# binli123/dsmil-wsi

Measured on NVIDIA H100. Metric: patches/sec DSMIL fwd at N=10k D=512, higher is better.
Workload: dtype f32

## Files before the change

dsmil_wsi_b200/csrc/abi.cu:

```cuda
#include <atomic>
#include <cstdarg>
#include <cstdio>
#include <cstring>
#include <cstdlib>
#include <vector>
#include <algorithm>
#include <climits>

#include "common.cuh"
#include "gemm_generic.cuh"
#include "fwd_kernels.cuh"
#include "bwd_kernels.cuh"
#include "bwd_bags.cuh"
#include "fwd_sm90.cuh"
#include "fwd_batched.cuh"
#include "bag_plan.cuh"
#include "embed_kernels.cuh"
#include "jpeg_kernels.cuh"

namespace dsmil {

static thread_local char g_err[512] = "";
__device__ unsigned long long scratch_keys[kMaxC];
static std::atomic<uint64_t> g_launches{0};

void set_error(const char* fmt, ...) {
  va_list ap;
  va_start(ap, fmt);
  vsnprintf(g_err, sizeof(g_err), fmt, ap);
  va_end(ap);
}
int cuda_fail(cudaError_t e, const char* what) {
  set_error("CUDA error %d (%s) at %s", static_cast<int>(e), cudaGetErrorString(e), what);
  return DSMIL_ERR_CUDA;
}
void count_launch(int n) { g_launches.fetch_add(static_cast<uint64_t>(n), std::memory_order_relaxed); }

__global__ void __launch_bounds__(256)
k_gather_rows(const float* __restrict__ X, int D, const long long* __restrict__ idx, long long M,
              float* __restrict__ out) {
  const int lane = threadIdx.x & 31;
  const long long stride = static_cast<long long>(gridDim.x) * 8;
  const bool vec = (D % 4 == 0) && ((reinterpret_cast<uintptr_t>(X) & 15) == 0) && ((reinterpret_cast<uintptr_t>(out) & 15) == 0);
  for (long long m = static_cast<long long>(blockIdx.x) * 8 + (threadIdx.x >> 5); m < M; m += stride) {
    const float* src = X + idx[m] * D;
    float* dst = out + m * D;
    if (vec) {
      for (int j = lane; j < (D >> 2); j += 32)
        reinterpret_cast<float4*>(dst)[j] = __ldg(reinterpret_cast<const float4*>(src) + j);
    } else {
      for (int j = lane; j < D; j += 32) dst[j] = __ldg(src + j);
    }
  }
}



__global__ void __launch_bounds__(256)
k_u8hwc_to_f32chw(const uint8_t* __restrict__ in, long long B, int H, int W, int Cc, float* __restrict__ out) {
  const long long plane = static_cast<long long>(H) * W;
  const long long total = B * plane;
  const long long stride = static_cast<long long>(gridDim.x) * blockDim.x;
  for (long long i = static_cast<long long>(blockIdx.x) * blockDim.x + threadIdx.x; i < total; i += stride) {
    const long long b = i / plane, px = i % plane;
    const uint8_t* src = in + i * Cc;
    float* dst = out + b * Cc * plane + px;
    for (int c = 0; c < Cc; ++c) dst[c * plane] = __fdiv_rn(static_cast<float>(src[c]), 255.f);
  }
}

bool g_prof_on = false;
struct ProfRec { int tag; cudaEvent_t a, b; };
static std::vector<ProfRec> g_prof;
static std::vector<ProfRec> g_prof_pool;
static int g_prof_open[PROF_NTAGS];
void prof_begin_impl(int tag, cudaStream_t st) {
  if (g_prof.size() >= 16384) { g_prof_open[tag] = -1; return; }
  ProfRec r;
  if (!g_prof_pool.empty()) { r = g_prof_pool.back(); g_prof_pool.pop_back(); }
  else { if (cudaEventCreate(&r.a) != cudaSuccess || cudaEventCreate(&r.b) != cudaSuccess) { g_prof_open[tag] = -1; return; } }
  r.tag = tag;
  cudaEventRecord(r.a, st);
  g_prof_open[tag] = static_cast<int>(g_prof.size());
  g_prof.push_back(r);
}
void prof_end_impl(int tag, cudaStream_t st) {
  const int i = g_prof_open[tag];
  if (i >= 0 && i < static_cast<int>(g_prof.size())) cudaEventRecord(g_prof[i].b, st);
}

static int check_params(const dsmil_params_t* p, bool need_scores = false) {
  DSMIL_REQUIRE(p != nullptr, "params is NULL");
  DSMIL_REQUIRE(!need_scores || (p->Wi && p->bi), "NULL instance-classifier weights");
  DSMIL_REQUIRE(p->D >= 1 && p->D <= DSMIL_MAX_D, "feature size D=%d outside [1,%d]", p->D, DSMIL_MAX_D);
  DSMIL_REQUIRE(p->C >= 1 && p->C <= DSMIL_MAX_C, "output classes C=%d outside [1,%d]", p->C, DSMIL_MAX_C);
  DSMIL_REQUIRE(p->W1 && p->b1 && p->Wf && p->bf, "NULL weight pointer");
  DSMIL_REQUIRE(!p->nonlinear || (p->W2 && p->b2), "nonlinear q needs W2/b2");
  DSMIL_REQUIRE(!p->passing_v || (p->Wv && p->bv), "passing_v needs Wv/bv");
  return 0;
}

static int check_workspace(size_t need, bool ok, const void* ws, size_t cap) {
  if (ws && ok) return 0;
  set_error("workspace too small: need %zu bytes, got %zu", need, cap);
  return DSMIL_ERR_WORKSPACE;
}

static int check_bags(const float* const* Xs, const int64_t* Ns, int nb, int64_t* total, bool* aligned) {
  *total = 0;
  *aligned = true;
  for (int b = 0; b < nb; ++b) {
    DSMIL_REQUIRE(Ns[b] >= 0 && Ns[b] < 0xffffffffll, "bag %d: N=%lld out of range", b, (long long)Ns[b]);
    if (Ns[b] == 0) {
      set_error("bag %d: empty bag (N == 0): the reference raises IndexError at dsmil.py:53", b);
      return DSMIL_ERR_EMPTY;
    }
    if (!Xs) {
      *total += Ns[b];
      continue;
    }
    DSMIL_REQUIRE(Xs[b], "bag %d: NULL features", b);
    *aligned = *aligned && (reinterpret_cast<uintptr_t>(Xs[b]) & 15) == 0;
    *total += Ns[b];
  }
  return 0;
}

static inline int attend_ctas(int64_t N) {
  const int64_t tiles = (N + kAttendRows - 1) / kAttendRows;
  return static_cast<int>(tiles < kSplits ? (tiles < 1 ? 1 : tiles) : kSplits);
}

static int num_sms() {
  static int cached[64] = {0};
  int dev = 0;
  if (cudaGetDevice(&dev) != cudaSuccess || dev < 0 || dev >= 64) return kSms;
  if (!cached[dev]) {
    int n = 0;
    if (cudaDeviceGetAttribute(&n, cudaDevAttrMultiProcessorCount, dev) != cudaSuccess || n <= 0) n = kSms;
    cached[dev] = n;
  }
  return cached[dev];
}

struct Phase1Ws {
  sm90::BagDev* table;
  unsigned long long* keys;
  unsigned int* counters;
  uint8_t* wimg;
};
static void carve_phase1(Carver& c, const dsmil_params_t* p, int nb, Phase1Ws& w) {
  w.table = c.take<sm90::BagDev>(nb);
  w.keys = c.take<unsigned long long>(static_cast<size_t>(nb) * (kMaxC + 1));
  w.counters = reinterpret_cast<unsigned int*>(w.keys ? w.keys + static_cast<size_t>(nb) * kMaxC : nullptr);
  w.wimg = nullptr;
  if (sm90::qmlp_supported(p)) {
    const uintptr_t img = reinterpret_cast<uintptr_t>(c.take<uint8_t>(sm90::wimg_bytes(p->D) + 1024));
    w.wimg = reinterpret_cast<uint8_t*>((img + 1023) & ~uintptr_t(1023));
  }
}

static int build_table(const float* const* Xs, const int64_t* Ns, int nb, std::vector<sm90::BagDev>& tbl, int* tiles,
                       int* recs) {
  long long row = 0;
  int tile = 0, rec = 0;
  tbl.resize(nb);
  for (int b = 0; b < nb; ++b) {
    DSMIL_REQUIRE(Ns[b] >= 1 && Ns[b] < 0xffffffffll && Xs[b], "bag %d: empty or NULL", b);
    DSMIL_REQUIRE((reinterpret_cast<uintptr_t>(Xs[b]) & 15) == 0, "bag %d: features must be 16-byte aligned", b);
    tbl[b] = bag_entry(Xs[b], Ns[b], row, tile, rec);
  }
  *tiles = tile;
  *recs = rec;
  return 0;
}

static int bags_phase1_impl(const dsmil_params_t* p, const Phase1Ws& w, const float* const* Xs, const int64_t* Ns,
                            int nb, const float* classes_in, float* classes, float* Q, float* H1, bool q_blocked,
                            bool upload, int* tiles, int* recs, cudaStream_t st) {
  std::vector<sm90::BagDev> tbl;
  int rc;
  if ((rc = build_table(Xs, Ns, nb, tbl, tiles, recs))) return rc;
  if (upload)
    DSMIL_CUDA_OK(cudaMemcpyAsync(w.table, tbl.data(), sizeof(sm90::BagDev) * nb, cudaMemcpyHostToDevice, st));
  DSMIL_CUDA_OK(cudaMemsetAsync(w.keys, 0, sizeof(unsigned long long) * (kMaxC + 1) * nb, st));
  if (upload && (rc = sm90::launch_prep_wimg(p, w.wimg, st))) return rc;
  if (classes_in) {
    const int grid = static_cast<int>(std::min<int64_t>(ceil_div(Ns[0], 256), kSplits));
    k_argmax<<<grid, 256, 0, st>>>(classes_in, Ns[0], p->C, w.keys);
    DSMIL_LAUNCH_OK("k_argmax");
  }
  return sm90::launch_qmlp(p, w.table, nb, *tiles, classes_in ? nullptr : classes, w.keys, Q, H1, w.wimg, num_sms(),
                           st, q_blocked);
}

struct FwdWs : Phase1Ws {
  float *Q, *H1, *V, *cand, *qmax, *recs, *rec;
  int64_t* crit;
  size_t bytes;
};
static FwdWs carve_fwd(const dsmil_params_t* p, int64_t N, void* ws, size_t cap, bool* ok) {
  Carver c(ws, cap);
  FwdWs w;
  const int64_t n = N > 0 ? N : 1;
  carve_phase1(c, p, 1, w);
  w.Q = c.take<float>(n * kQ);
  w.H1 = p->nonlinear ? c.take<float>(n * kQ) : nullptr;
  w.V = p->passing_v ? c.take<float>(n * p->D) : nullptr;
  w.cand = c.take<float>(cand_floats(p->C));
  w.qmax = c.take<float>(static_cast<size_t>(p->C) * kQ);
  w.crit = c.take<int64_t>(kMaxC);
  w.recs = c.take<float>(static_cast<size_t>(attend_ctas(N)) * rec_floats(p->C, p->D));
  w.rec = c.take<float>(rec_floats(p->C, p->D));
  w.bytes = c.off;
  *ok = c.ok();
  return w;
}


static int launch_scores(const dsmil_params_t* p, const float* X, int64_t N, float* classes,
                         unsigned long long* keys, cudaStream_t st) {
  const int C = p->C, D = p->D;
  const size_t smem = sizeof(float) * C * D;
  const bool vec = (D % 4 == 0) && ((reinterpret_cast<uintptr_t>(X) & 15) == 0);
  const int mode = !vec ? 0 : (D % 64 == 0 ? 2 : 1);
  const int grid = static_cast<int>(std::min<int64_t>(ceil_div(N, mode == 2 ? 64 : 8), kSms * 8));
  prof_begin(PROF_SCORES, st);
  if (mode == 2) {
    if (smem > 48 * 1024) DSMIL_CUDA_OK(cudaFuncSetAttribute(k_scores<2>, cudaFuncAttributeMaxDynamicSharedMemorySize, (int)smem));
    k_scores<2><<<grid, 256, smem, st>>>(X, N, D, p->Wi, p->bi, C, classes, keys);
  } else if (mode == 1) {
    if (smem > 48 * 1024) DSMIL_CUDA_OK(cudaFuncSetAttribute(k_scores<1>, cudaFuncAttributeMaxDynamicSharedMemorySize, (int)smem));
    k_scores<1><<<grid, 256, smem, st>>>(X, N, D, p->Wi, p->bi, C, classes, keys);
  } else {
    if (smem > 48 * 1024) DSMIL_CUDA_OK(cudaFuncSetAttribute(k_scores<0>, cudaFuncAttributeMaxDynamicSharedMemorySize, (int)smem));
    k_scores<0><<<grid, 256, smem, st>>>(X, N, D, p->Wi, p->bi, C, classes, keys);
  }
  prof_end(PROF_SCORES, st);
  DSMIL_LAUNCH_OK("k_scores");
  return 0;
}

static bool stream_is_capturing(cudaStream_t st) {
  cudaStreamCaptureStatus cs = cudaStreamCaptureStatusNone;
  return cudaStreamIsCapturing(st, &cs) == cudaSuccess && cs != cudaStreamCaptureStatusNone;
}

static bool phase1_on_qmlp(const dsmil_params_t* p, const uint8_t* wimg, const float* X) {
  return sm90::qmlp_supported(p) && wimg && (reinterpret_cast<uintptr_t>(X) & 15) == 0;
}

static int phase1_impl(const dsmil_params_t* p, const float* X, const float* xv, const float* classes_in,
                       int64_t N, int64_t row_offset, float* classes, float* Q, float* H1, float* V,
                       float* cand, const Phase1Ws& w, cudaStream_t st) {
  const int C = p->C, D = p->D;
  int rc;
  if (N > 0 && classes_in && classes && classes != classes_in)
    DSMIL_CUDA_OK(cudaMemcpyAsync(classes, classes_in, sizeof(float) * N * C, cudaMemcpyDeviceToDevice, st));
  if (N > 0 && phase1_on_qmlp(p, w.wimg, X)) {
    int tiles, recs;
    if ((rc = bags_phase1_impl(p, w, &X, &N, 1, classes_in, classes, Q, H1, false, true, &tiles, &recs, st))) return rc;
  } else {
    DSMIL_CUDA_OK(cudaMemsetAsync(w.keys, 0, sizeof(unsigned long long) * kMaxC, st));
    if (N > 0) {
      if (classes_in) {
        const int grid = static_cast<int>(std::min<int64_t>(ceil_div(N, 256), kSplits));
        k_argmax<<<grid, 256, 0, st>>>(classes_in, N, C, w.keys);
        DSMIL_LAUNCH_OK("k_argmax");
      } else if ((rc = launch_scores(p, X, N, classes, w.keys, st))) {
        return rc;
      }
      prof_begin(PROF_QMLP, st);
      if (p->nonlinear) {
        if ((rc = launch_linear<ACT_RELU, false>(X, N, D, p->W1, p->b1, kQ, H1, nullptr, 0, st))) return rc;
        if ((rc = launch_linear<ACT_TANH, false>(H1, N, kQ, p->W2, p->b2, kQ, Q, nullptr, 0, st))) return rc;
      } else {
        if ((rc = launch_linear<ACT_NONE, false>(X, N, D, p->W1, p->b1, kQ, Q, nullptr, 0, st))) return rc;
      }
      prof_end(PROF_QMLP, st);
    }
  }
  if (N > 0 && p->passing_v &&
      (rc = launch_linear<ACT_RELU, false>(xv ? xv : X, N, D, p->Wv, p->bv, D, V, nullptr, 0, st)))
    return rc;
  const float* cls = classes_in ? classes_in : classes;
  k_gather_cand<<<C, kQ, 0, st>>>(w.keys, cls, Q, N, C, row_offset, cand);
  DSMIL_LAUNCH_OK("k_gather_cand");
  return 0;
}

__global__ void k_empty_rec(float* rec, int C, int Dv) {
  const size_t n = rec_floats(C, Dv);
  for (size_t i = blockIdx.x * blockDim.x + threadIdx.x; i < n; i += static_cast<size_t>(gridDim.x) * blockDim.x)
    rec[i] = (i < static_cast<size_t>(C)) ? -INFINITY : 0.f;
}

template <int CT>
static int launch_attend_j(int J, int grid, cudaStream_t st, const float* V, int Dv, const float* Q, int64_t N,
                           const float* qmax, int C, float* A, float* recs) {
  switch (J) {
    case 1: k_attend<CT, 1><<<grid, 256, 0, st>>>(V, Dv, Q, N, qmax, C, A, recs); break;
    case 2: k_attend<CT, 2><<<grid, 256, 0, st>>>(V, Dv, Q, N, qmax, C, A, recs); break;
    case 4: k_attend<CT, 4><<<grid, 256, 0, st>>>(V, Dv, Q, N, qmax, C, A, recs); break;
    case 8: k_attend<CT, 8><<<grid, 256, 0, st>>>(V, Dv, Q, N, qmax, C, A, recs); break;
    default: k_attend<CT, 16><<<grid, 256, 0, st>>>(V, Dv, Q, N, qmax, C, A, recs); break;
  }
  DSMIL_LAUNCH_OK("k_attend");
  return 0;
}

static int phase2_impl(const dsmil_params_t* p, const float* V, const float* Q, int64_t N, const float* qmax,
                       float* A, float* rec, float* recs, cudaStream_t st) {
  const int C = p->C, Dv = p->D;
  if (N <= 0) {
    k_empty_rec<<<4, 256, 0, st>>>(rec, C, Dv);
    DSMIL_LAUNCH_OK("k_empty_rec");
    return 0;
  }
  const int grid = attend_ctas(N);
  int j = ceil_div(Dv, 256), J = 1;
  while (J < j) J <<= 1;
  int rc;
  prof_begin(PROF_ATTEND, st);
  if (C == 1) rc = launch_attend_j<1>(J, grid, st, V, Dv, Q, N, qmax, C, A, recs);
  else if (C == 2) rc = launch_attend_j<2>(J, grid, st, V, Dv, Q, N, qmax, C, A, recs);
  else if (C <= 4) rc = launch_attend_j<4>(J, grid, st, V, Dv, Q, N, qmax, C, A, recs);
  else rc = launch_attend_j<8>(J, grid, st, V, Dv, Q, N, qmax, C, A, recs);
  prof_end(PROF_ATTEND, st);
  if (rc) return rc;
  dim3 g2(C, ceil_div(Dv, 256));
  k_combine_rec<<<g2, 256, 0, st>>>(recs, grid, C, Dv, rec);
  DSMIL_LAUNCH_OK("k_combine_rec");
  return 0;
}

static int phase3_impl(const dsmil_params_t* p, int64_t N, const float* rec, float* A, float* B, float* pred,
                       cudaStream_t st) {
  const int grid = static_cast<int>(std::min<int64_t>(std::max<int64_t>(ceil_div(N * p->C, 256), 1), kSplits));
  prof_begin(PROF_FINAL, st);
  k_finalize<<<grid, 256, 0, st>>>(rec, N, p->C, p->D, p->Wf, p->bf, A, B, pred);
  prof_end(PROF_FINAL, st);
  DSMIL_LAUNCH_OK("k_finalize");
  return 0;
}

static int forward_bags_impl(const dsmil_params_t* p, const float* const* Xs, const int64_t* Ns, int nb,
                             const float* classes_in, float* classes, float* pred, float* A, float* B,
                             int64_t* crit, float* save_Q, float* save_H1, void* ws, size_t ws_bytes,
                             cudaStream_t st);

static int forward_impl(const dsmil_params_t* p, const float* X, const float* xv, const float* classes_in,
                        int64_t N, float* classes, float* pred, float* A, float* B, int64_t* crit_idx,
                        float* save_Q, float* save_H1, float* save_V, void* ws, size_t ws_bytes, cudaStream_t st) {
  int rc = check_params(p, classes_in == nullptr);
  if (rc) return rc;
  DSMIL_REQUIRE(N >= 0 && N < 0xffffffffll, "N=%lld out of range", (long long)N);
  if (N == 0) {
    set_error("empty bag (N == 0): the reference raises IndexError at dsmil.py:53");
    return DSMIL_ERR_EMPTY;
  }
  DSMIL_REQUIRE(X && pred && A && B && (classes || classes_in), "NULL tensor pointer");
  if (sm90::batched_supported(p) && (reinterpret_cast<uintptr_t>(X) & 15) == 0)
    return forward_bags_impl(p, &X, &N, 1, classes_in, classes, pred, A, B, crit_idx, save_Q, save_H1, ws, ws_bytes, st);
  bool ok;
  FwdWs w = carve_fwd(p, N, ws, ws_bytes, &ok);
  if ((rc = check_workspace(w.bytes, ok, ws, ws_bytes))) return rc;
  float* Q = save_Q ? save_Q : w.Q;
  float* H1 = p->nonlinear ? (save_H1 ? save_H1 : w.H1) : nullptr;
  float* V = p->passing_v ? (save_V ? save_V : w.V) : nullptr;
  if ((rc = phase1_impl(p, X, xv, classes_in, N, 0, classes, Q, H1, V, w.cand, w, st))) return rc;
  int64_t* crit = crit_idx ? crit_idx : w.crit;
  k_merge_cand<<<p->C, kQ, 0, st>>>(w.cand, 1, 1, p->C, w.qmax, crit);
  DSMIL_LAUNCH_OK("k_merge_cand");
  const float* Vv = p->passing_v ? V : X;
  if ((rc = phase2_impl(p, Vv, Q, N, w.qmax, A, w.rec, w.recs, st))) return rc;
  return phase3_impl(p, N, w.rec, A, B, pred, st);
}


struct BagsWs : Phase1Ws {
  float* Q;
  float* recs;
  float* pred_part;
  long long* row_offsets;
  float* qmax;
  size_t bytes;
};
static BagsWs carve_bags(const dsmil_params_t* p, const int64_t* Ns, int nb, bool need_Q, bool sharded, void* ws,
                         size_t cap, bool* ok) {
  Carver c(ws, cap);
  BagsWs w;
  int64_t tiles = 0, nrec = 0;
  for (int b = 0; b < nb; ++b) {
    tiles += tiles_for_bag(Ns[b]);
    nrec += recs_for_bag(Ns[b]);
  }
  carve_phase1(c, p, nb, w);
  w.pred_part = c.take<float>(static_cast<size_t>(nb) * sm90::kFinSlices * kMaxC);
  w.Q = need_Q ? c.take<float>(static_cast<size_t>(tiles) * sm90::kTileM * kQ) : nullptr;
  w.recs = c.take<float>(static_cast<size_t>(nrec) * rec_floats(p->C, p->D));
  w.row_offsets = sharded ? c.take<long long>(nb) : nullptr;
  w.qmax = sharded ? c.take<float>(static_cast<size_t>(nb) * p->C * kQ) : nullptr;
  w.bytes = c.off;
  *ok = c.ok();
  return w;
}

static int bags_attend_finalize(const dsmil_params_t* p, const BagsWs& w, int nb, const float* Q, bool q_blocked,
                                float* pred, float* A, float* B, int64_t* crit, int recs, const int* recs_dev,
                                cudaStream_t st) {
  const int C = p->C, D = p->D;
  int rc;
  sm90::AttendArgs aa{w.table, nb, D, C, Q, q_blocked, w.keys, A, w.recs, nullptr, recs_dev};
  if ((rc = sm90::launch_attend_b(aa, recs, st))) return rc;
  sm90::FinalizeArgs fa{w.table, D, C, w.recs, w.keys, p->Wf, p->bf, A, B, pred, reinterpret_cast<long long*>(crit),
                         w.pred_part, w.counters, nullptr, 0, 0};
  return sm90::launch_finalize_b(fa, nb, st);
}

static int forward_bags_impl(const dsmil_params_t* p, const float* const* Xs, const int64_t* Ns, int nb,
                             const float* classes_in, float* classes, float* pred, float* A, float* B,
                             int64_t* crit, float* save_Q, float* save_H1, void* ws, size_t ws_bytes,
                             cudaStream_t st) {
  bool ok;
  BagsWs w = carve_bags(p, Ns, nb, save_Q == nullptr, false, ws, ws_bytes, &ok);
  int rc = check_workspace(w.bytes, ok, ws, ws_bytes);
  if (rc) return rc;
  float* Q = save_Q ? save_Q : w.Q;
  const bool q_blocked = save_Q == nullptr;
  int tiles, recs;
  if ((rc = bags_phase1_impl(p, w, Xs, Ns, nb, classes_in, classes, Q, save_H1, q_blocked, true, &tiles, &recs, st)))
    return rc;
  return bags_attend_finalize(p, w, nb, Q, q_blocked, pred, A, B, crit, recs, nullptr, st);
}

}

using namespace dsmil;

extern "C" {

int dsmil_abi_version(void) { return DSMIL_ABI_VERSION; }
const char* dsmil_last_error(void) { return g_err; }
uint64_t dsmil_launch_count(void) { return g_launches.load(std::memory_order_relaxed); }
int dsmil_forward_path(const dsmil_params_t* p, int64_t N) {
  (void)N;
  return (p && p->C >= 1 && p->C <= DSMIL_MAX_C && p->D >= 1 && p->D <= DSMIL_MAX_D && sm90::qmlp_supported(p)) ? 2 : 1;
}


int dsmil_gather_rows(const float* X, int64_t N, int32_t D, const int64_t* idx, int64_t M, float* out, void* stream) {
  DSMIL_REQUIRE(N >= 0 && M >= 0 && D >= 1 && (M == 0 || (X && idx && out)), "bad arguments");
  if (M == 0) return 0;
  const int grid = static_cast<int>(std::min<int64_t>((M + 7) / 8, kSms * 8));
  k_gather_rows<<<grid, 256, 0, static_cast<cudaStream_t>(stream)>>>(X, D, reinterpret_cast<const long long*>(idx), M, out);
  DSMIL_LAUNCH_OK("k_gather_rows");
  return 0;
}

int dsmil_patches_u8_to_f32(const uint8_t* in, int64_t B, int32_t H, int32_t W, int32_t Cc, float* out, void* stream) {
  DSMIL_REQUIRE(B >= 0 && H >= 1 && W >= 1 && Cc >= 1 && Cc <= 4 && (B == 0 || (in && out)), "bad arguments");
  if (B == 0) return 0;
  const long long total = static_cast<long long>(B) * H * W;
  const int grid = static_cast<int>(std::min<long long>((total + 255) / 256, kSms * 16));
  k_u8hwc_to_f32chw<<<grid, 256, 0, static_cast<cudaStream_t>(stream)>>>(in, B, H, W, Cc, out);
  DSMIL_LAUNCH_OK("k_u8hwc_to_f32chw");
  return 0;
}

int dsmil_instnorm_act(const float* x, const float* residual, float* y, int64_t planes, int32_t HW, float eps,
                       int32_t relu, void* stream) {
  DSMIL_REQUIRE(planes >= 0 && HW >= 1 && HW <= kInPlaneMax && eps >= 0.f && (planes == 0 || (x && y)),
                "bad arguments (HW must be in [1, %d])", kInPlaneMax);
  DSMIL_REQUIRE(planes < (1ll << 31), "too many planes");
  if (planes == 0) return 0;
  return launch_instnorm(x, residual, y, planes, HW, eps, relu, static_cast<cudaStream_t>(stream));
}

int dsmil_instnorm_act_nhwc(const float* x, const float* residual, float* y, int64_t N, int32_t HW, int32_t C, float eps,
                            int32_t relu, void* stream) {
  DSMIL_REQUIRE(N >= 0 && HW >= 1 && C >= 32 && C % 32 == 0 && eps >= 0.f && (N == 0 || (x && y)),
                "bad arguments (C must be a multiple of 32)");
  DSMIL_REQUIRE(N * (C / 32) < (1ll << 31), "too many (sample, channel group) slabs");
  if (N == 0) return 0;
  return launch_instnorm_nhwc(x, residual, y, N, HW, C, eps, relu, static_cast<cudaStream_t>(stream));
}

static JpegBatch carve_jpeg(void* ws, size_t cap, int n, int H, int W, int64_t blob_bytes, size_t* need) {
  Carver cv(ws, cap);
  JpegBatch a{};
  a.n = n; a.H = H; a.W = W;
  a.plane_elems = jpeg_plane_elems(H, W);
  a.unstuffed = cv.take<uint8_t>(static_cast<size_t>(blob_bytes) + 64);
  a.coef = cv.take<int16_t>(static_cast<size_t>(3) * a.plane_elems * n);
  a.planes = cv.take<uint8_t>(static_cast<size_t>(3) * a.plane_elems * n);
  *need = cv.off;
  return a;
}

int32_t dsmil_jpeg_header_bytes_dev(void) { return static_cast<int32_t>(sizeof(dsmil_jpeg_header)); }

int64_t dsmil_jpeg_workspace_bytes(int32_t n, int32_t H, int32_t W, int64_t blob_bytes) {
  if (n < 0 || H < 1 || W < 1 || H > 65535 || W > 65535 || blob_bytes < 0) return -1;
  size_t need = 0;
  carve_jpeg(nullptr, 0, n, H, W, blob_bytes, &need);
  return static_cast<int64_t>(need);
}

int dsmil_jpeg_decode_batch(const uint8_t* blob, int64_t blob_bytes, const void* headers, int32_t n, int32_t H, int32_t W,
                            uint8_t* out_u8, float* out_f32, int32_t f32_channels_last, int32_t* status, void* workspace,
                            int64_t workspace_bytes, void* stream) {
  DSMIL_REQUIRE(n >= 0 && H >= 1 && W >= 1 && H <= 65535 && W <= 65535 && blob_bytes >= 0 &&
                (f32_channels_last == 0 || f32_channels_last == 1), "bad arguments");
  if (n == 0) return 0;
  DSMIL_REQUIRE(blob && headers && status && workspace && (out_u8 || out_f32), "null pointer");
  DSMIL_REQUIRE((reinterpret_cast<uintptr_t>(headers) & 15) == 0 && (reinterpret_cast<uintptr_t>(workspace) & 255) == 0 &&
                (out_f32 == nullptr || (reinterpret_cast<uintptr_t>(out_f32) & 15) == 0) &&
                (out_u8 == nullptr || (reinterpret_cast<uintptr_t>(out_u8) & 3) == 0),
                "headers must be 16-byte, workspace 256-byte, out_f32 16-byte, out_u8 4-byte aligned");
  size_t need = 0;
  JpegBatch a = carve_jpeg(workspace, static_cast<size_t>(workspace_bytes), n, H, W, blob_bytes, &need);
  const int rc = check_workspace(need, static_cast<int64_t>(need) <= workspace_bytes, workspace,
                                 static_cast<size_t>(std::max<int64_t>(workspace_bytes, 0)));
  if (rc) return rc;
  a.blob = blob;
  a.hdr = static_cast<const dsmil_jpeg_header*>(headers);
  a.out_u8 = out_u8;
  a.out_f32 = out_f32;
  a.f32_hwc = f32_channels_last;
  a.status = status;
  return launch_jpeg_decode(a, static_cast<cudaStream_t>(stream));
}

int dsmil_profile_enable(int on) {
  g_prof_on = on != 0;
  return 0;
}
int dsmil_profile_read(double* ms_per_tag, uint64_t* launches_per_tag) {
  DSMIL_REQUIRE(ms_per_tag && launches_per_tag, "NULL output");
  for (int t = 0; t < PROF_NTAGS; ++t) { ms_per_tag[t] = 0.0; launches_per_tag[t] = 0; }
  for (auto& r : g_prof) {
    float ms = 0.f;
    if (cudaEventSynchronize(r.b) == cudaSuccess && cudaEventElapsedTime(&ms, r.a, r.b) == cudaSuccess) {
      ms_per_tag[r.tag] += ms;
      launches_per_tag[r.tag] += 1;
    }
    g_prof_pool.push_back(r);
  }
  g_prof.clear();
  cudaGetLastError();
  return 0;
}

size_t dsmil_cand_floats(int32_t C) { return cand_floats(C); }
size_t dsmil_rec_floats(int32_t C, int32_t Dv) { return rec_floats(C, Dv); }

size_t dsmil_forward_workspace_bytes(const dsmil_params_t* p, int64_t N) {
  if (!p || p->C < 1 || p->C > DSMIL_MAX_C || p->D < 1 || p->D > DSMIL_MAX_D || N < 0) return 0;
  bool ok;
  size_t a = carve_fwd(p, N, nullptr, 0, &ok).bytes;
  if (sm90::batched_supported(p) && N > 0) a = std::max(a, carve_bags(p, &N, 1, true, false, nullptr, 0, &ok).bytes);
  return a;
}

size_t dsmil_forward_bags_workspace_bytes(const dsmil_params_t* p, const int64_t* Ns, int32_t nb) {
  if (!p || !Ns || nb < 1 || p->C < 1 || p->C > DSMIL_MAX_C || p->D < 1 || p->D > DSMIL_MAX_D) return 0;
  bool ok;
  int64_t mx = 0;
  for (int b = 0; b < nb; ++b) mx = std::max<int64_t>(mx, Ns[b]);
  size_t bytes = carve_fwd(p, mx, nullptr, 0, &ok).bytes;
  if (sm90::batched_supported(p)) bytes = std::max(bytes, carve_bags(p, Ns, nb, true, false, nullptr, 0, &ok).bytes);
  return bytes;
}

int dsmil_forward_bags(const dsmil_params_t* p, const float* const* Xs, const int64_t* Ns, int32_t nb,
                       float* classes, float* pred, float* A, float* B, int64_t* crit_idx, void* workspace,
                       size_t workspace_bytes, void* stream) {
  int rc = check_params(p, true);
  if (rc) return rc;
  DSMIL_REQUIRE(Xs && Ns && nb >= 1 && classes && pred && A && B, "NULL pointer or nb < 1");
  cudaStream_t st = static_cast<cudaStream_t>(stream);
  int64_t total;
  bool aligned;
  if ((rc = check_bags(Xs, Ns, nb, &total, &aligned))) return rc;
  const size_t need = dsmil_forward_bags_workspace_bytes(p, Ns, nb);
  if ((rc = check_workspace(need, workspace_bytes >= need, workspace, workspace ? workspace_bytes : 0))) return rc;
  if (sm90::batched_supported(p) && aligned)
    return forward_bags_impl(p, Xs, Ns, nb, nullptr, classes, pred, A, B, crit_idx, nullptr, nullptr, workspace,
                             workspace_bytes, st);
  int64_t row = 0;
  for (int b = 0; b < nb; ++b) {
    rc = forward_impl(p, Xs[b], nullptr, nullptr, Ns[b], classes + row * p->C, pred + static_cast<size_t>(b) * p->C,
                      A + row * p->C, B + static_cast<size_t>(b) * p->C * p->D,
                      crit_idx ? crit_idx + static_cast<size_t>(b) * p->C : nullptr, nullptr, nullptr, nullptr,
                      workspace, workspace_bytes, st);
    if (rc) return rc;
    row += Ns[b];
  }
  return 0;
}
size_t dsmil_shard_workspace_bytes(const dsmil_params_t* p, int64_t N_local) {
  return dsmil_forward_workspace_bytes(p, N_local);
}

int dsmil_forward(const dsmil_params_t* p, const float* X, const float* x_for_v, int64_t N, float* classes,
                  float* pred, float* A, float* B, int64_t* crit_idx, float* save_Q, float* save_H1,
                  float* save_V, void* workspace, size_t workspace_bytes, void* stream) {
  DSMIL_REQUIRE(classes != nullptr, "classes is NULL");
  return forward_impl(p, X, x_for_v, nullptr, N, classes, pred, A, B, crit_idx, save_Q, save_H1, save_V,
                      workspace, workspace_bytes, static_cast<cudaStream_t>(stream));
}

int dsmil_bag_forward(const dsmil_params_t* p, const float* X, const float* x_for_v, const float* classes_in,
                      int64_t N, float* pred, float* A, float* B, int64_t* crit_idx, float* save_Q,
                      float* save_H1, float* save_V, void* workspace, size_t workspace_bytes, void* stream) {
  DSMIL_REQUIRE(classes_in != nullptr, "classes_in is NULL");
  return forward_impl(p, X, x_for_v, classes_in, N, nullptr, pred, A, B, crit_idx, save_Q, save_H1, save_V,
                      workspace, workspace_bytes, static_cast<cudaStream_t>(stream));
}

int dsmil_instance_scores(const dsmil_params_t* p, const float* X, int64_t N, float* classes, void* stream) {
  DSMIL_REQUIRE(p && p->Wi && p->bi && p->C >= 1 && p->C <= DSMIL_MAX_C && p->D >= 1 && p->D <= DSMIL_MAX_D,
                "bad params");
  DSMIL_REQUIRE(N >= 0 && (N == 0 || (X && classes)), "NULL tensor pointer");
  if (N == 0) return 0;
  unsigned long long* keys;
  DSMIL_CUDA_OK(cudaGetSymbolAddress(reinterpret_cast<void**>(&keys), scratch_keys));
  return launch_scores(p, X, N, classes, keys, static_cast<cudaStream_t>(stream));
}

int dsmil_shard_phase1(const dsmil_params_t* p, const float* X, const float* x_for_v, const float* classes_in,
                       int64_t N_local, int64_t row_offset, float* classes, float* Q, float* H1, float* V,
                       float* cand_rec, void* workspace, size_t workspace_bytes, void* stream) {
  int rc = check_params(p, classes_in == nullptr);
  if (rc) return rc;
  DSMIL_REQUIRE(N_local >= 0 && N_local < 0xffffffffll, "N_local out of range");
  DSMIL_REQUIRE(cand_rec && (N_local == 0 || (X && Q && (classes || classes_in))), "NULL tensor pointer");
  DSMIL_REQUIRE(N_local == 0 || !p->passing_v || V, "passing_v needs a V buffer");
  bool ok;
  FwdWs w = carve_fwd(p, N_local, workspace, workspace_bytes, &ok);
  if ((rc = check_workspace(w.bytes, ok, workspace, workspace_bytes))) return rc;
  float* h1 = p->nonlinear ? (H1 ? H1 : (phase1_on_qmlp(p, w.wimg, X) ? nullptr : w.H1)) : nullptr;
  return phase1_impl(p, X, x_for_v, classes_in, N_local, row_offset, classes, Q, h1, V, cand_rec, w,
                     static_cast<cudaStream_t>(stream));
}

int dsmil_shard_merge_candidates(int32_t C, const float* cand_recs, int32_t G, float* q_max, int64_t* crit_idx,
                                 void* stream) {
  DSMIL_REQUIRE(C >= 1 && C <= DSMIL_MAX_C && G >= 1 && cand_recs && q_max && crit_idx, "bad arguments");
  k_merge_cand<<<C, kQ, 0, static_cast<cudaStream_t>(stream)>>>(cand_recs, G, 1, C, q_max, crit_idx);
  DSMIL_LAUNCH_OK("k_merge_cand");
  return 0;
}

int dsmil_shard_phase2(const dsmil_params_t* p, const float* Xv, const float* Q, int64_t N_local,
                       const float* q_max, float* A_logits, float* rec, void* workspace, size_t workspace_bytes,
                       void* stream) {
  int rc = check_params(p);
  if (rc) return rc;
  DSMIL_REQUIRE(rec && q_max && (N_local == 0 || (Xv && Q && A_logits)), "NULL tensor pointer");
  bool ok;
  FwdWs w = carve_fwd(p, N_local, workspace, workspace_bytes, &ok);
  if ((rc = check_workspace(w.bytes, ok, workspace, workspace_bytes))) return rc;
  return phase2_impl(p, Xv, Q, N_local, q_max, A_logits, rec, w.recs, static_cast<cudaStream_t>(stream));
}

int dsmil_shard_merge_partials(int32_t C, int32_t Dv, const float* recs, int32_t G, float* rec_out, void* stream) {
  DSMIL_REQUIRE(C >= 1 && C <= DSMIL_MAX_C && Dv >= 1 && G >= 1 && G <= kMaxRecs && recs && rec_out, "bad arguments");
  dim3 g2(C, ceil_div(Dv, 256));
  k_combine_rec<<<g2, 256, 0, static_cast<cudaStream_t>(stream)>>>(recs, G, C, Dv, rec_out);
  DSMIL_LAUNCH_OK("k_combine_rec");
  return 0;
}

int dsmil_shard_phase3(const dsmil_params_t* p, int64_t N_local, const float* rec_global, float* A, float* B,
                       float* pred, void* stream) {
  int rc = check_params(p);
  if (rc) return rc;
  DSMIL_REQUIRE(rec_global && B && pred && (N_local == 0 || A), "NULL tensor pointer");
  return phase3_impl(p, N_local, rec_global, A, B, pred, static_cast<cudaStream_t>(stream));
}

struct BwdWs {
  float *dB, *dA, *tpart, *dqm, *dz2, *dz1, *tnpart, *cspart, *dzv, *tmp;
  size_t bytes;
};
static BwdWs carve_bwd(const dsmil_params_t* p, int64_t N, int need_gX, void* ws, size_t cap, bool* ok) {
  Carver c(ws, cap);
  BwdWs w;
  const int C = p->C, D = p->D;
  const int64_t n = N > 0 ? N : 1;
  w.dB = c.take<float>(static_cast<size_t>(C) * D);
  w.dA = c.take<float>(n * C);
  w.tpart = c.take<float>(kSplits * kMaxC);
  w.dqm = c.take<float>(static_cast<size_t>(C) * kQ);
  w.dz2 = c.take<float>(n * kQ);
  w.dz1 = p->nonlinear ? c.take<float>(n * kQ) : nullptr;
  size_t tn = tn_partial_floats(kQ, D, N);
  tn = std::max(tn, tn_partial_floats(kQ, kQ, N));
  tn = std::max(tn, tn_partial_floats(C, kQ, N));
  tn = std::max(tn, tn_partial_floats(C, D, N));
  if (p->passing_v) tn = std::max(tn, tn_partial_floats(D, D, N));
  w.tnpart = c.take<float>(tn);
  w.cspart = c.take<float>(static_cast<size_t>(kSplits) * std::max(D, kQ));
  w.dzv = p->passing_v ? c.take<float>(n * D) : nullptr;
  w.tmp = (p->passing_v && need_gX) ? c.take<float>(n * D) : nullptr;
  w.bytes = c.off;
  *ok = c.ok();
  return w;
}

size_t dsmil_backward_workspace_bytes(const dsmil_params_t* p, int64_t N, int need_gX) {
  if (!p || p->C < 1 || p->C > DSMIL_MAX_C || p->D < 1 || p->D > DSMIL_MAX_D || N < 0) return 0;
  bool ok;
  return carve_bwd(p, N, need_gX, nullptr, 0, &ok).bytes;
}


static int bwd_phase1_impl(const dsmil_params_t* p, const float* X, const float* Vv, int64_t N, const float* A,
                           const float* B, const float* d_classes, const float* d_pred, const float* d_A,
                           const float* d_B, const dsmil_grads_t* g, float* dA, const BwdWs& w, int* gs,
                           cudaStream_t st) {
  const int C = p->C, D = p->D;
  int rc;
  k_bwd_bag<<<ceil_div(static_cast<int64_t>(C) * D, 256), 256, 0, st>>>(p->Wf, B, d_pred, d_B, C, D, w.dB, g->gWf,
                                                                        g->gbf);
  DSMIL_LAUNCH_OK("k_bwd_bag");
  if (g->gWi) {
    if (d_classes && N > 0) { if ((rc = launch_gemm_tn(d_classes, C, X, D, N, w.tnpart, g->gWi, st))) return rc; }
    else DSMIL_CUDA_OK(cudaMemsetAsync(g->gWi, 0, sizeof(float) * C * D, st));
  }
  if (g->gbi) {
    if (d_classes && N > 0) { if ((rc = launch_colsum(d_classes, C, N, w.cspart, g->gbi, st))) return rc; }
    else DSMIL_CUDA_OK(cudaMemsetAsync(g->gbi, 0, sizeof(float) * C, st));
  }
  *gs = static_cast<int>(std::min<int64_t>(ceil_div(N, 256), kSplits));
  if (N == 0) return 0;
  const size_t smem = sizeof(float) * C * D;
  if (smem > 48 * 1024)
    DSMIL_CUDA_OK(cudaFuncSetAttribute(k_rowdot, cudaFuncAttributeMaxDynamicSharedMemorySize, (int)smem));
  const int grid = static_cast<int>(std::min<int64_t>(ceil_div(N, 8), kSms * 8));
  k_rowdot<<<grid, 256, smem, st>>>(Vv, N, D, w.dB, C, d_A, dA);
  DSMIL_LAUNCH_OK("k_rowdot");
  k_bwd_t_partial<<<*gs, 256, 0, st>>>(A, dA, N, C, w.tpart);
  DSMIL_LAUNCH_OK("k_bwd_t_partial");
  return 0;
}

static int bwd_phase2_impl(const dsmil_params_t* p, int64_t N, const float* A, float* dA, const float* part, int P,
                           const float* Q, float* dqm, const BwdWs& w, cudaStream_t st) {
  if (N > 0) {
    const int gs = static_cast<int>(std::min<int64_t>(ceil_div(N, 256), kSplits));
    k_bwd_dL<<<gs, 256, 0, st>>>(A, dA, N, p->C, part, P);
    DSMIL_LAUNCH_OK("k_bwd_dL");
  }
  return launch_gemm_tn(dA, p->C, Q, kQ, N, w.tnpart, dqm, st);
}

static int bwd_phase3_impl(const dsmil_params_t* p, const float* X, int64_t N, int64_t row_offset, const float* Q,
                           const float* H1, const float* dL, const float* dqm, const float* qmax, const int64_t* crit,
                           const dsmil_grads_t* g, const BwdWs& w, const float** dz1, cudaStream_t st) {
  int rc;
  if (N > 0) {
    const int grid = static_cast<int>(std::min<int64_t>(ceil_div(N * kQ, 256), kSms * 8));
    k_bwd_dq<<<grid, 256, 0, st>>>(dL, Q, qmax, dqm, crit, N, row_offset, p->C, p->nonlinear, w.dz2);
    DSMIL_LAUNCH_OK("k_bwd_dq");
  }
  *dz1 = w.dz2;
  if (p->nonlinear) {
    if (g->gW2 && (rc = launch_gemm_tn(w.dz2, kQ, H1, kQ, N, w.tnpart, g->gW2, st))) return rc;
    if (g->gb2 && (rc = launch_colsum(w.dz2, kQ, N, w.cspart, g->gb2, st))) return rc;
    if (N > 0 && (rc = launch_linear<ACT_MASK_POS, true>(w.dz2, N, kQ, p->W2, nullptr, kQ, w.dz1, H1, 0, st))) return rc;
    *dz1 = w.dz1;
  }
  if (g->gW1 && (rc = launch_gemm_tn(*dz1, kQ, X, p->D, N, w.tnpart, g->gW1, st))) return rc;
  if (g->gb1 && (rc = launch_colsum(*dz1, kQ, N, w.cspart, g->gb1, st))) return rc;
  return 0;
}

int dsmil_backward(const dsmil_params_t* p, const float* X, const float* x_for_v, int64_t N, const float* Q,
                   const float* H1, const float* V, const float* A, const float* B, const int64_t* crit_idx,
                   const float* d_classes, const float* d_pred, const float* d_A, const float* d_B,
                   const dsmil_grads_t* g, const float* v_mask, void* workspace, size_t workspace_bytes,
                   void* stream) {
  int rc = check_params(p);
  if (rc) return rc;
  DSMIL_REQUIRE(N >= 1 && X && Q && A && B && crit_idx && g, "NULL tensor pointer or N < 1");
  DSMIL_REQUIRE(!p->nonlinear || H1, "nonlinear q backward needs saved H1");
  DSMIL_REQUIRE(!p->passing_v || V, "passing_v backward needs saved V");
  cudaStream_t st = static_cast<cudaStream_t>(stream);
  const int C = p->C, D = p->D;
  bool ok;
  BwdWs w = carve_bwd(p, N, g->gX != nullptr, workspace, workspace_bytes, &ok);
  if ((rc = check_workspace(w.bytes, ok, workspace, workspace_bytes))) return rc;
  const float* Xv = x_for_v ? x_for_v : X;
  int gs;
  const float* dz1;
  if ((rc = bwd_phase1_impl(p, X, p->passing_v ? V : X, N, A, B, d_classes, d_pred, d_A, d_B, g, w.dA, w, &gs, st)) ||
      (rc = bwd_phase2_impl(p, N, A, w.dA, w.tpart, gs, Q, w.dqm, w, st)) ||
      (rc = bwd_phase3_impl(p, X, N, 0, Q, H1, w.dA, w.dqm, nullptr, crit_idx, g, w, &dz1, st)))
    return rc;

  const int ge = static_cast<int>(std::min<int64_t>(ceil_div(N * D, 256), kSms * 8));
  if (p->passing_v) {
    k_bwd_dzv<<<ge, 256, 0, st>>>(A, w.dB, V, N, C, D, w.dzv);
    DSMIL_LAUNCH_OK("k_bwd_dzv");
    if (g->gWv && (rc = launch_gemm_tn(w.dzv, D, Xv, D, N, w.tnpart, g->gWv, st))) return rc;
    if (g->gbv && (rc = launch_colsum(w.dzv, D, N, w.cspart, g->gbv, st))) return rc;
  }
  if (g->gX) {
    if ((rc = launch_linear<ACT_NONE, true>(dz1, N, kQ, p->W1, nullptr, D, g->gX, nullptr, 0, st))) return rc;
    k_bwd_dx_extra<<<ge, 256, 0, st>>>(d_classes, p->Wi, p->passing_v ? nullptr : A, w.dB, N, C, D, 1, g->gX);
    DSMIL_LAUNCH_OK("k_bwd_dx_extra");
    if (p->passing_v) {
      if ((rc = launch_linear<ACT_NONE, true>(w.dzv, N, D, p->Wv, nullptr, D, w.tmp, nullptr, 0, st))) return rc;
      k_axpy_mask<<<ge, 256, 0, st>>>(w.tmp, v_mask, N * D, g->gX);
      DSMIL_LAUNCH_OK("k_axpy_mask");
    }
  }
  return 0;
}

int dsmil_shard_backward_phase1(const dsmil_params_t* p, const float* X, int64_t N, const float* A, const float* B,
                                const float* d_classes, const float* d_pred, float* dA, float* t_local, float* gWi,
                                float* gbi, float* gWf, float* gbf, void* workspace, size_t workspace_bytes,
                                void* stream) {
  int rc = check_params(p);
  if (rc) return rc;
  DSMIL_REQUIRE(!p->passing_v, "sharded backward supports the identity v only");
  DSMIL_REQUIRE(N >= 0 && B && t_local && (N == 0 || (X && A && dA)), "NULL tensor pointer or N < 0");
  cudaStream_t st = static_cast<cudaStream_t>(stream);
  bool ok;
  BwdWs w = carve_bwd(p, N, 0, workspace, workspace_bytes, &ok);
  if ((rc = check_workspace(w.bytes, ok, workspace, workspace_bytes))) return rc;
  dsmil_grads_t g{};
  g.gWi = gWi; g.gbi = gbi; g.gWf = gWf; g.gbf = gbf;
  int gs;
  if ((rc = bwd_phase1_impl(p, X, X, N, A, B, d_classes, d_pred, nullptr, nullptr, &g, dA, w, &gs, st))) return rc;
  if (N == 0) {
    DSMIL_CUDA_OK(cudaMemsetAsync(t_local, 0, sizeof(float) * p->C, st));
    return 0;
  }
  return launch_sum_partials(w.tpart, gs, p->C, t_local, st);
}

int dsmil_shard_backward_phase2(const dsmil_params_t* p, int64_t N, const float* A, float* dA, const float* t_global,
                                const float* Q, float* dqm_local, void* workspace, size_t workspace_bytes,
                                void* stream) {
  int rc = check_params(p);
  if (rc) return rc;
  DSMIL_REQUIRE(N >= 0 && t_global && dqm_local && (N == 0 || (A && dA && Q)), "NULL tensor pointer or N < 0");
  bool ok;
  BwdWs w = carve_bwd(p, N, 0, workspace, workspace_bytes, &ok);
  if ((rc = check_workspace(w.bytes, ok, workspace, workspace_bytes))) return rc;
  return bwd_phase2_impl(p, N, A, dA, t_global, 1, Q, dqm_local, w, static_cast<cudaStream_t>(stream));
}

int dsmil_shard_backward_phase3(const dsmil_params_t* p, const float* X, int64_t N, int64_t row_offset, const float* Q,
                                const float* H1, const float* dL, const float* dqm_global, const float* q_max,
                                const int64_t* crit_idx, float* gW1, float* gb1, float* gW2, float* gb2,
                                void* workspace, size_t workspace_bytes, void* stream) {
  int rc = check_params(p);
  if (rc) return rc;
  DSMIL_REQUIRE(N >= 0 && dqm_global && q_max && crit_idx && (N == 0 || (X && Q && dL)), "NULL tensor pointer or N < 0");
  DSMIL_REQUIRE(!p->nonlinear || N == 0 || H1, "nonlinear q backward needs saved H1");
  bool ok;
  BwdWs w = carve_bwd(p, N, 0, workspace, workspace_bytes, &ok);
  if ((rc = check_workspace(w.bytes, ok, workspace, workspace_bytes))) return rc;
  dsmil_grads_t g{};
  g.gW1 = gW1; g.gb1 = gb1; g.gW2 = gW2; g.gb2 = gb2;
  const float* dz1;
  return bwd_phase3_impl(p, X, N, row_offset, Q, H1, dL, dqm_global, q_max, crit_idx, &g, w, &dz1,
                         static_cast<cudaStream_t>(stream));
}

int dsmil_instance_scores_backward(const dsmil_params_t* p, const float* X, int64_t N, const float* d_classes,
                                   float* gWi, float* gbi, float* gX, void* workspace, size_t workspace_bytes,
                                   void* stream) {
  DSMIL_REQUIRE(p && p->Wi && p->C >= 1 && p->C <= DSMIL_MAX_C && p->D >= 1 && p->D <= DSMIL_MAX_D, "bad params");
  DSMIL_REQUIRE(N >= 1 && X && d_classes, "NULL tensor pointer or N < 1");
  cudaStream_t st = static_cast<cudaStream_t>(stream);
  const int C = p->C, D = p->D;
  Carver c(workspace, workspace_bytes);
  float* tnpart = c.take<float>(tn_partial_floats(C, D, N));
  float* cspart = c.take<float>(static_cast<size_t>(kSplits) * kMaxC);
  int rc = check_workspace(c.off, c.ok(), workspace, workspace_bytes);
  if (rc) return rc;
  if (gWi && (rc = launch_gemm_tn(d_classes, C, X, D, N, tnpart, gWi, st))) return rc;
  if (gbi && (rc = launch_colsum(d_classes, C, N, cspart, gbi, st))) return rc;
  if (gX) {
    const int ge = static_cast<int>(std::min<int64_t>(ceil_div(N * D, 256), kSms * 8));
    k_bwd_dx_extra<<<ge, 256, 0, st>>>(d_classes, p->Wi, nullptr, nullptr, N, C, D, 0, gX);
    DSMIL_LAUNCH_OK("k_bwd_dx_extra");
  }
  return 0;
}

struct BwdBagsWs {
  BagsPlan* plan;
  float* zero_row;
  sm90::BagDev* table;
  TnChunk *chi, *ch1;
  float *dB, *dA, *dL, *tpart, *dpart, *dqm, *dz2, *dz1, *tnpart, *cspart;
  long long* row_offsets;
  int G;
  bool gemv_i;
  int nci, nc1;
  int64_t rps_i, rps_1;
  size_t bytes;
};
static void layout_bwd_bags(Carver& c, const dsmil_params_t* p, int nb, int64_t n, int nchi, bool sharded,
                            BwdBagsWs& w) {
  const int C = p->C, D = p->D;
  w.table = c.take<sm90::BagDev>(nb);
  w.chi = c.take<TnChunk>(nchi);
  w.ch1 = c.take<TnChunk>(w.nc1);
  w.dB = c.take<float>(static_cast<size_t>(nb) * C * D);
  w.dA = c.take<float>(n * C);
  w.dL = c.take<float>(n * C);
  w.tpart = c.take<float>(static_cast<size_t>(nb) * w.G * C);
  w.dpart = c.take<float>(static_cast<size_t>(nb) * w.G * C * kQ);
  w.dqm = c.take<float>(static_cast<size_t>(nb) * C * kQ);
  w.dz2 = c.take<float>(n * kQ);
  w.dz1 = p->nonlinear ? c.take<float>(n * kQ) : nullptr;
  size_t tn = static_cast<size_t>(nchi) * C * D;
  tn = std::max(tn, static_cast<size_t>(w.nc1) * kQ * D);
  tn = std::max(tn, tn_partial_floats(kQ, kQ, n));
  w.tnpart = c.take<float>(tn);
  w.cspart = c.take<float>(static_cast<size_t>(kSplits) * kQ);
  w.row_offsets = sharded ? c.take<long long>(nb) : nullptr;
}
static BwdBagsWs carve_bwd_bags(const dsmil_params_t* p, const int64_t* Ns, int nb, bool aligned, bool sharded,
                                void* ws, size_t cap, bool* ok) {
  Carver c(ws, cap);
  BwdBagsWs w;
  const int C = p->C, D = p->D;
  int64_t total = 0, mx = 1;
  for (int b = 0; b < nb; ++b) {
    total += Ns[b];
    mx = std::max<int64_t>(mx, Ns[b]);
  }
  w.plan = nullptr;
  w.zero_row = nullptr;
  w.G = bwd_bags_ctas(nb, mx);
  const bool gemv_ok = tn_use_gemv(C, D);
  w.gemv_i = gemv_ok && aligned;
  const int64_t rps_gemv = rag_rows_per_chunk(C, D, total, true), rps_tile = rag_rows_per_chunk(C, D, total, false);
  const int nci_gemv = gemv_ok ? rag_chunks(nullptr, Ns, nb, D, rps_gemv, nullptr) : 0;
  const int nci_tile = rag_chunks(nullptr, Ns, nb, D, rps_tile, nullptr);
  w.rps_i = w.gemv_i ? rps_gemv : rps_tile;
  w.nci = w.gemv_i ? nci_gemv : nci_tile;
  w.rps_1 = rag_rows_per_chunk(kQ, D, total, false);
  w.nc1 = rag_chunks(nullptr, Ns, nb, D, w.rps_1, nullptr);
  layout_bwd_bags(c, p, nb, std::max<int64_t>(total, 1), std::max(nci_gemv, nci_tile), sharded, w);
  w.bytes = c.off;
  *ok = c.ok();
  return w;
}
static BwdBagsWs carve_bwd_bags_dev(const dsmil_params_t* p, int nb, int64_t max_rows, void* ws, size_t cap,
                                    bool* ok) {
  Carver c(ws, cap);
  BwdBagsWs w;
  const int C = p->C, D = p->D;
  w.G = bwd_bags_ctas(nb, max_rows);
  w.gemv_i = tn_use_gemv(C, D);
  w.nci = rag_chunks_cap(C, D, w.gemv_i, nb);
  w.nc1 = rag_chunks_cap(kQ, D, false, nb);
  w.rps_i = w.rps_1 = 0;
  layout_bwd_bags(c, p, nb, static_cast<int64_t>(nb) * max_rows, w.nci, false, w);
  w.plan = c.take<BagsPlan>(1);
  w.zero_row = c.take<float>(D);
  w.bytes = c.off;
  *ok = c.ok();
  return w;
}


static int bwd_bags_phase1_impl(const dsmil_params_t* p, const float* const* Xs, const int64_t* Ns, int nb,
                                int64_t total, const float* A, const float* B, const float* d_classes,
                                const float* d_pred, const float* d_A, const float* d_B, const dsmil_grads_t* g,
                                float* dA, const BwdBagsWs& w, cudaStream_t st) {
  const int C = p->C, D = p->D;
  const BagsPlan* pl = w.plan;
  int rc;
  if (!pl) {
    std::vector<sm90::BagDev> tbl(nb);
    long long row = 0;
    for (int b = 0; b < nb; ++b) {
      tbl[b] = sm90::BagDev{Xs[b], Ns[b], row, 0, 0, 0, 0};
      row += Ns[b];
    }
    std::vector<TnChunk> chi(w.nci), ch1(w.nc1);
    rag_chunks(Xs, Ns, nb, D, w.rps_i, chi.data());
    rag_chunks(Xs, Ns, nb, D, w.rps_1, ch1.data());
    DSMIL_CUDA_OK(cudaMemcpyAsync(w.table, tbl.data(), sizeof(sm90::BagDev) * nb, cudaMemcpyHostToDevice, st));
    DSMIL_CUDA_OK(cudaMemcpyAsync(w.chi, chi.data(), sizeof(TnChunk) * w.nci, cudaMemcpyHostToDevice, st));
    DSMIL_CUDA_OK(cudaMemcpyAsync(w.ch1, ch1.data(), sizeof(TnChunk) * w.nc1, cudaMemcpyHostToDevice, st));
  }

  k_bwd_bag_b<<<ceil_div(static_cast<int64_t>(C) * D, 256), 256, 0, st>>>(p->Wf, B, d_pred, d_B, nb, C, D, w.dB,
                                                                          g->gWf, g->gbf);
  DSMIL_LAUNCH_OK("k_bwd_bag_b");
  if (g->gWi) {
    if (d_classes) {
      if ((rc = launch_gemm_tn_rag(d_classes, C, D, w.chi, w.nci, w.gemv_i, w.tnpart, g->gWi, st, pl ? &pl->nci : nullptr)))
        return rc;
    }
    else DSMIL_CUDA_OK(cudaMemsetAsync(g->gWi, 0, sizeof(float) * C * D, st));
  }
  if (g->gbi) {
    if (d_classes) { if ((rc = launch_colsum(d_classes, C, total, w.cspart, g->gbi, st, pl ? &pl->cs : nullptr))) return rc; }
    else DSMIL_CUDA_OK(cudaMemsetAsync(g->gbi, 0, sizeof(float) * C, st));
  }
  const size_t smem = sizeof(float) * C * D;
  if (smem > 48 * 1024)
    DSMIL_CUDA_OK(cudaFuncSetAttribute(k_bwd_rowdot_b, cudaFuncAttributeMaxDynamicSharedMemorySize, (int)smem));
  k_bwd_rowdot_b<<<dim3(w.G, nb), 256, smem, st>>>(w.table, D, w.dB, C, A, d_A, dA, w.tpart, pl ? &pl->G : nullptr);
  DSMIL_LAUNCH_OK("k_bwd_rowdot_b");
  return 0;
}

static int bwd_bags_phase2_impl(const dsmil_params_t* p, int nb, const float* A, const float* dA, const float* tpart,
                                int P, const float* Q, float* dL, float* dqm, const BwdBagsWs& w, cudaStream_t st) {
  const int C = p->C;
  const int* G_dev = w.plan ? &w.plan->G : nullptr;
  k_bwd_dL_b<<<dim3(w.G, nb), 256, 0, st>>>(w.table, C, A, dA, tpart, P, Q, dL, w.dpart, G_dev);
  DSMIL_LAUNCH_OK("k_bwd_dL_b");
  k_sum_segments<<<dim3(ceil_div(C * kQ, 256), nb), 256, 0, st>>>(w.dpart, w.G, C * kQ, dqm, G_dev);
  DSMIL_LAUNCH_OK("k_sum_segments");
  return 0;
}

static int bwd_bags_phase3_impl(const dsmil_params_t* p, int nb, int64_t total, const float* Q, const float* H1,
                                const float* dL, const float* dqm, const float* qmax, const int64_t* crit,
                                const long long* row_offsets, const dsmil_grads_t* g, const BwdBagsWs& w,
                                const float** dz1, cudaStream_t st) {
  const int D = p->D;
  const BagsPlan* pl = w.plan;
  int rc;
  k_bwd_dq_b<<<dim3(w.G, nb), 256, 0, st>>>(w.table, p->C, dL, Q, qmax, dqm, crit, row_offsets, p->nonlinear, w.dz2);
  DSMIL_LAUNCH_OK("k_bwd_dq_b");
  *dz1 = w.dz2;
  if (p->nonlinear) {
    if (g->gW2 && (rc = launch_gemm_tn(w.dz2, kQ, H1, kQ, total, w.tnpart, g->gW2, st, pl ? &pl->tn2 : nullptr)))
      return rc;
    if (g->gb2 && (rc = launch_colsum(w.dz2, kQ, total, w.cspart, g->gb2, st, pl ? &pl->cs : nullptr))) return rc;
    if ((rc = launch_linear<ACT_MASK_POS, true>(w.dz2, total, kQ, p->W2, nullptr, kQ, w.dz1, H1, 0, st,
                                                pl ? &pl->total : nullptr)))
      return rc;
    *dz1 = w.dz1;
  }
  if (g->gW1 &&
      (rc = launch_gemm_tn_rag(*dz1, kQ, D, w.ch1, w.nc1, false, w.tnpart, g->gW1, st, pl ? &pl->nc1 : nullptr)))
    return rc;
  if (g->gb1 && (rc = launch_colsum(*dz1, kQ, total, w.cspart, g->gb1, st, pl ? &pl->cs : nullptr))) return rc;
  return 0;
}

static int backward_bags_run(const dsmil_params_t* p, const float* const* Xs, const int64_t* Ns, int nb, int64_t total,
                             const float* Q, const float* H1, const float* A, const float* B, const int64_t* crit,
                             const float* d_classes, const float* d_pred, const float* d_A, const float* d_B,
                             const dsmil_grads_t* g, const BwdBagsWs& w, cudaStream_t st) {
  const int C = p->C, D = p->D;
  int rc;
  const float* dz1;
  if ((rc = bwd_bags_phase1_impl(p, Xs, Ns, nb, total, A, B, d_classes, d_pred, d_A, d_B, g, w.dA, w, st)) ||
      (rc = bwd_bags_phase2_impl(p, nb, A, w.dA, w.tpart, w.G, Q, w.dL, w.dqm, w, st)) ||
      (rc = bwd_bags_phase3_impl(p, nb, total, Q, H1, w.dL, w.dqm, nullptr, crit, nullptr, g, w, &dz1, st)))
    return rc;
  if (g->gX) {
    if ((rc = launch_linear<ACT_NONE, true>(dz1, total, kQ, p->W1, nullptr, D, g->gX, nullptr, 0, st))) return rc;
    k_bwd_dx_extra_b<<<dim3(w.G, nb), 256, 0, st>>>(w.table, d_classes, p->Wi, A, w.dB, C, D, g->gX);
    DSMIL_LAUNCH_OK("k_bwd_dx_extra_b");
  }
  return 0;
}

static int backward_bags_impl(const dsmil_params_t* p, const float* const* Xs, const int64_t* Ns, int nb,
                              int64_t total, bool aligned, const float* Q, const float* H1, const float* A,
                              const float* B, const int64_t* crit, const float* d_classes, const float* d_pred,
                              const float* d_A, const float* d_B, const dsmil_grads_t* g, void* ws, size_t ws_bytes,
                              cudaStream_t st) {
  bool ok;
  BwdBagsWs w = carve_bwd_bags(p, Ns, nb, aligned, false, ws, ws_bytes, &ok);
  int rc = check_workspace(w.bytes, ok, ws, ws_bytes);
  if (rc) return rc;
  return backward_bags_run(p, Xs, Ns, nb, total, Q, H1, A, B, crit, d_classes, d_pred, d_A, d_B, g, w, st);
}

int dsmil_shard_bags_supported(const dsmil_params_t* p) {
  return (p && p->C >= 1 && p->C <= DSMIL_MAX_C && p->D >= 1 && p->D <= DSMIL_MAX_D && sm90::batched_supported(p)) ? 1 : 0;
}
size_t dsmil_shard_bags_workspace_bytes(const dsmil_params_t* p, const int64_t* Ns, int32_t nb) {
  if (!dsmil_shard_bags_supported(p) || !Ns || nb < 1) return 0;
  bool ok;
  return carve_bags(p, Ns, nb, true, true, nullptr, 0, &ok).bytes;
}
static int shard_bags_phase1_impl(const dsmil_params_t* p, const float* const* Xs, const int64_t* Ns, int nb,
                                  const int64_t* row_offsets, float* classes, float* Q, float* H1, bool q_blocked,
                                  float* cand_recs, const BagsWs& w, cudaStream_t st) {
  const bool upload = !stream_is_capturing(st);
  int tiles, recs, rc;
  if ((rc = bags_phase1_impl(p, w, Xs, Ns, nb, nullptr, classes, Q, H1, q_blocked, upload, &tiles, &recs, st)))
    return rc;
  if (upload)
    DSMIL_CUDA_OK(cudaMemcpyAsync(w.row_offsets, row_offsets, sizeof(long long) * nb, cudaMemcpyHostToDevice, st));
  sm90::k_gather_cand_b<<<dim3(p->C, nb), kQ, 0, st>>>(w.table, w.keys, classes, Q, q_blocked, w.row_offsets, p->C,
                                                        cand_recs);
  DSMIL_LAUNCH_OK("k_gather_cand_b");
  return 0;
}
static int shard_bags_phase2_impl(const dsmil_params_t* p, const float* const* Xs, const int64_t* Ns, int nb,
                                  const float* Q, bool q_blocked, const float* cands_all, int G, float* A,
                                  int64_t* crit_idx, float* qmax, float* recs_out, const BagsWs& w, cudaStream_t st) {
  std::vector<sm90::BagDev> tbl;
  int tiles = 0, recs = 0, rc;
  if ((rc = build_table(Xs, Ns, nb, tbl, &tiles, &recs))) return rc;
  k_merge_cand<<<dim3(p->C, nb), kQ, 0, st>>>(cands_all, G, nb, p->C, qmax, crit_idx);
  DSMIL_LAUNCH_OK("k_merge_cand");
  sm90::AttendArgs aa{w.table, nb, p->D, p->C, Q, q_blocked, w.keys, A, w.recs, qmax, nullptr};
  if ((rc = sm90::launch_attend_b(aa, recs, st))) return rc;
  sm90::FinalizeArgs fa{w.table, p->D, p->C, w.recs, w.keys, p->Wf, p->bf, A, nullptr, nullptr, nullptr,
                         w.pred_part, w.counters, recs_out, 0, 0};
  return sm90::launch_finalize_b(fa, nb, st);
}

int dsmil_shard_bags_phase1(const dsmil_params_t* p, const float* const* Xs, const int64_t* Ns, int32_t nb,
                            const int64_t* row_offsets, float* classes, float* cand_recs, void* workspace,
                            size_t workspace_bytes, void* stream) {
  int rc = check_params(p, true);
  if (rc) return rc;
  DSMIL_REQUIRE(dsmil_shard_bags_supported(p), "shape not supported by the batched tensor-core path");
  DSMIL_REQUIRE(Xs && Ns && nb >= 1 && row_offsets && classes && cand_recs, "NULL pointer or nb < 1");
  bool ok;
  BagsWs w = carve_bags(p, Ns, nb, true, true, workspace, workspace_bytes, &ok);
  if ((rc = check_workspace(w.bytes, ok, workspace, workspace_bytes))) return rc;
  return shard_bags_phase1_impl(p, Xs, Ns, nb, row_offsets, classes, w.Q, nullptr, true, cand_recs, w,
                                static_cast<cudaStream_t>(stream));
}
int dsmil_shard_bags_phase2(const dsmil_params_t* p, const float* const* Xs, const int64_t* Ns, int32_t nb,
                            const float* cands_all, int32_t G, float* A, int64_t* crit_idx, float* recs_out,
                            void* workspace, size_t workspace_bytes, void* stream) {
  int rc = check_params(p, true);
  if (rc) return rc;
  DSMIL_REQUIRE(dsmil_shard_bags_supported(p) && Xs && Ns && nb >= 1 && cands_all && G >= 1 && A && crit_idx && recs_out,
                "bad arguments");
  bool ok;
  BagsWs w = carve_bags(p, Ns, nb, true, true, workspace, workspace_bytes, &ok);
  if ((rc = check_workspace(w.bytes, ok, workspace, workspace_bytes))) return rc;
  return shard_bags_phase2_impl(p, Xs, Ns, nb, w.Q, true, cands_all, G, A, crit_idx, w.qmax, recs_out, w,
                                static_cast<cudaStream_t>(stream));
}
int dsmil_shard_bags_phase3(const dsmil_params_t* p, const float* const* Xs, const int64_t* Ns, int32_t nb,
                            const float* recs_all, int32_t G, float* A, float* B, float* pred, void* workspace,
                            size_t workspace_bytes, void* stream) {
  int rc = check_params(p, true);
  if (rc) return rc;
  DSMIL_REQUIRE(dsmil_shard_bags_supported(p) && Xs && Ns && nb >= 1 && recs_all && G >= 1 && G <= sm90::kMaxRecPerBag && A && B && pred,
                "bad arguments");
  cudaStream_t st = static_cast<cudaStream_t>(stream);
  bool ok;
  BagsWs w = carve_bags(p, Ns, nb, true, true, workspace, workspace_bytes, &ok);
  if ((rc = check_workspace(w.bytes, ok, workspace, workspace_bytes))) return rc;
  sm90::FinalizeArgs fa{w.table, p->D, p->C, recs_all, w.keys, p->Wf, p->bf, A, B, pred, nullptr,
                         w.pred_part, w.counters, nullptr, G, nb};
  return sm90::launch_finalize_b(fa, nb, st);
}


size_t dsmil_forward_bags_train_workspace_bytes(const dsmil_params_t* p, const int64_t* Ns, int32_t nb) {
  if (!p || p->passing_v) return 0;
  return dsmil_forward_bags_workspace_bytes(p, Ns, nb);
}

int dsmil_forward_bags_train(const dsmil_params_t* p, const float* const* Xs, const int64_t* Ns, int32_t nb,
                             float* classes, float* pred, float* A, float* B, int64_t* crit_idx, float* save_Q,
                             float* save_H1, void* workspace, size_t workspace_bytes, void* stream) {
  int rc = check_params(p, true);
  if (rc) return rc;
  DSMIL_REQUIRE(!p->passing_v, "batched training supports the identity v only (passing_v: one bag per call)");
  DSMIL_REQUIRE(Xs && Ns && nb >= 1 && classes && pred && A && B && crit_idx && save_Q && (!p->nonlinear || save_H1),
                "NULL pointer or nb < 1");
  cudaStream_t st = static_cast<cudaStream_t>(stream);
  int64_t total;
  bool aligned;
  if ((rc = check_bags(Xs, Ns, nb, &total, &aligned))) return rc;
  const size_t need = dsmil_forward_bags_train_workspace_bytes(p, Ns, nb);
  if ((rc = check_workspace(need, workspace_bytes >= need, workspace, workspace ? workspace_bytes : 0))) return rc;
  if (sm90::batched_supported(p) && aligned)
    return forward_bags_impl(p, Xs, Ns, nb, nullptr, classes, pred, A, B, crit_idx, save_Q, save_H1, workspace,
                             workspace_bytes, st);
  int64_t row = 0;
  for (int b = 0; b < nb; ++b) {
    rc = forward_impl(p, Xs[b], nullptr, nullptr, Ns[b], classes + row * p->C, pred + static_cast<size_t>(b) * p->C,
                      A + row * p->C, B + static_cast<size_t>(b) * p->C * p->D, crit_idx + static_cast<size_t>(b) * p->C,
                      save_Q + row * kQ, save_H1 ? save_H1 + row * kQ : nullptr, nullptr, workspace, workspace_bytes,
                      st);
    if (rc) return rc;
    row += Ns[b];
  }
  return 0;
}

size_t dsmil_backward_bags_workspace_bytes(const dsmil_params_t* p, const int64_t* Ns, int32_t nb, int need_gX) {
  (void)need_gX;
  if (!p || !Ns || nb < 1 || p->passing_v || p->C < 1 || p->C > DSMIL_MAX_C || p->D < 1 || p->D > DSMIL_MAX_D) return 0;
  for (int b = 0; b < nb; ++b)
    if (Ns[b] < 0) return 0;
  bool ok;
  return carve_bwd_bags(p, Ns, nb, true, false, nullptr, 0, &ok).bytes;
}

int dsmil_backward_bags(const dsmil_params_t* p, const float* const* Xs, const int64_t* Ns, int32_t nb,
                        const float* Q, const float* H1, const float* A, const float* B, const int64_t* crit_idx,
                        const float* d_classes, const float* d_pred, const float* d_A, const float* d_B,
                        const dsmil_grads_t* grads, void* workspace, size_t workspace_bytes, void* stream) {
  int rc = check_params(p);
  if (rc) return rc;
  DSMIL_REQUIRE(!p->passing_v, "batched backward supports the identity v only (passing_v: dsmil_backward per bag)");
  DSMIL_REQUIRE(Xs && Ns && nb >= 1 && nb <= 65535 && Q && A && B && crit_idx && grads,
                "NULL pointer or nb outside [1, 65535]");
  DSMIL_REQUIRE(!p->nonlinear || H1, "nonlinear q backward needs saved H1");
  DSMIL_REQUIRE(!(grads->gX && d_classes) || p->Wi, "gX through d_classes needs Wi");
  int64_t total;
  bool aligned;
  if ((rc = check_bags(Xs, Ns, nb, &total, &aligned))) return rc;
  const size_t need = dsmil_backward_bags_workspace_bytes(p, Ns, nb, grads->gX != nullptr);
  if ((rc = check_workspace(need, workspace_bytes >= need, workspace, workspace ? workspace_bytes : 0))) return rc;
  return backward_bags_impl(p, Xs, Ns, nb, total, aligned, Q, H1, A, B, crit_idx, d_classes, d_pred, d_A, d_B, grads,
                            workspace, workspace_bytes, static_cast<cudaStream_t>(stream));
}


static int check_shard_bags_train(const dsmil_params_t* p, bool need_scores, const float* const* Xs, bool need_X,
                                  const int64_t* Ns, int nb, int64_t* total, bool* aligned) {
  int rc = check_params(p, need_scores);
  if (rc) return rc;
  DSMIL_REQUIRE(!p->passing_v, "row-sharded batched training supports the identity v only");
  DSMIL_REQUIRE(dsmil_shard_bags_supported(p), "shape not supported by the batched tensor-core path");
  DSMIL_REQUIRE(Ns && (Xs || !need_X) && nb >= 1 && nb <= 65535, "NULL pointer or nb outside [1, 65535]");
  return check_bags(need_X ? Xs : nullptr, Ns, nb, total, aligned);
}

int dsmil_shard_bags_phase1_train(const dsmil_params_t* p, const float* const* Xs, const int64_t* Ns, int32_t nb,
                                  const int64_t* row_offsets, float* classes, float* save_Q, float* save_H1,
                                  float* cand_recs, void* workspace, size_t workspace_bytes, void* stream) {
  int64_t total;
  bool aligned;
  int rc = check_shard_bags_train(p, true, Xs, true, Ns, nb, &total, &aligned);
  if (rc) return rc;
  DSMIL_REQUIRE(row_offsets && classes && save_Q && save_H1 && cand_recs, "NULL pointer");
  bool ok;
  BagsWs w = carve_bags(p, Ns, nb, true, true, workspace, workspace_bytes, &ok);
  if ((rc = check_workspace(w.bytes, ok, workspace, workspace_bytes))) return rc;
  return shard_bags_phase1_impl(p, Xs, Ns, nb, row_offsets, classes, save_Q, save_H1, false, cand_recs, w,
                                static_cast<cudaStream_t>(stream));
}

int dsmil_shard_bags_phase2_train(const dsmil_params_t* p, const float* const* Xs, const int64_t* Ns, int32_t nb,
                                  const float* Q, const float* cands_all, int32_t G, float* A, int64_t* crit_idx,
                                  float* q_max, float* recs_out, void* workspace, size_t workspace_bytes,
                                  void* stream) {
  int64_t total;
  bool aligned;
  int rc = check_shard_bags_train(p, true, Xs, true, Ns, nb, &total, &aligned);
  if (rc) return rc;
  DSMIL_REQUIRE(Q && cands_all && G >= 1 && A && crit_idx && q_max && recs_out, "NULL pointer or G < 1");
  bool ok;
  BagsWs w = carve_bags(p, Ns, nb, true, true, workspace, workspace_bytes, &ok);
  if ((rc = check_workspace(w.bytes, ok, workspace, workspace_bytes))) return rc;
  return shard_bags_phase2_impl(p, Xs, Ns, nb, Q, false, cands_all, G, A, crit_idx, q_max, recs_out, w,
                                static_cast<cudaStream_t>(stream));
}

size_t dsmil_shard_backward_bags_workspace_bytes(const dsmil_params_t* p, const int64_t* Ns, int32_t nb) {
  if (!dsmil_shard_bags_supported(p) || !Ns || nb < 1) return 0;
  for (int b = 0; b < nb; ++b)
    if (Ns[b] < 0) return 0;
  bool ok;
  return carve_bwd_bags(p, Ns, nb, true, true, nullptr, 0, &ok).bytes;
}

int dsmil_shard_backward_bags_phase1(const dsmil_params_t* p, const float* const* Xs, const int64_t* Ns, int32_t nb,
                                     const float* A, const float* B, const float* d_classes_local,
                                     const float* d_pred, float* dA_local, float* t_local, float* gWi, float* gbi,
                                     float* gWf, float* gbf, void* workspace, size_t workspace_bytes, void* stream) {
  int64_t total;
  bool aligned;
  int rc = check_shard_bags_train(p, false, Xs, true, Ns, nb, &total, &aligned);
  if (rc) return rc;
  DSMIL_REQUIRE(A && B && dA_local && t_local, "NULL tensor pointer");
  cudaStream_t st = static_cast<cudaStream_t>(stream);
  bool ok;
  BwdBagsWs w = carve_bwd_bags(p, Ns, nb, aligned, true, workspace, workspace_bytes, &ok);
  if ((rc = check_workspace(w.bytes, ok, workspace, workspace_bytes))) return rc;
  dsmil_grads_t g{};
  g.gWi = gWi; g.gbi = gbi; g.gWf = gWf; g.gbf = gbf;
  if ((rc = bwd_bags_phase1_impl(p, Xs, Ns, nb, total, A, B, d_classes_local, d_pred, nullptr, nullptr, &g, dA_local,
                                 w, st)))
    return rc;
  k_sum_segments<<<dim3(ceil_div(p->C, 256), nb), 256, 0, st>>>(w.tpart, w.G, p->C, t_local, nullptr);
  DSMIL_LAUNCH_OK("k_sum_segments");
  return 0;
}

int dsmil_shard_backward_bags_phase2(const dsmil_params_t* p, const int64_t* Ns, int32_t nb, const float* A,
                                     float* dA_to_dL, const float* t_global, const float* Q, float* dqm_local,
                                     void* workspace, size_t workspace_bytes, void* stream) {
  int64_t total;
  bool aligned;
  int rc = check_shard_bags_train(p, false, nullptr, false, Ns, nb, &total, &aligned);
  if (rc) return rc;
  DSMIL_REQUIRE(A && dA_to_dL && t_global && Q && dqm_local, "NULL tensor pointer");
  cudaStream_t st = static_cast<cudaStream_t>(stream);
  bool ok;
  BwdBagsWs w = carve_bwd_bags(p, Ns, nb, true, true, workspace, workspace_bytes, &ok);
  if ((rc = check_workspace(w.bytes, ok, workspace, workspace_bytes))) return rc;
  DSMIL_CUDA_OK(cudaMemcpyAsync(w.dA, dA_to_dL, sizeof(float) * total * p->C, cudaMemcpyDeviceToDevice, st));
  return bwd_bags_phase2_impl(p, nb, A, w.dA, t_global, 1, Q, dA_to_dL, dqm_local, w, st);
}

int dsmil_shard_backward_bags_phase3(const dsmil_params_t* p, const float* const* Xs, const int64_t* Ns, int32_t nb,
                                     const int64_t* row_offsets, const float* Q, const float* H1, const float* dL_local,
                                     const float* dqm_global, const float* q_max, const int64_t* crit_idx,
                                     float* gW1, float* gb1, float* gW2, float* gb2, void* workspace,
                                     size_t workspace_bytes, void* stream) {
  int64_t total;
  bool aligned;
  int rc = check_shard_bags_train(p, false, Xs, true, Ns, nb, &total, &aligned);
  if (rc) return rc;
  DSMIL_REQUIRE(row_offsets && Q && H1 && dL_local && dqm_global && q_max && crit_idx, "NULL tensor pointer");
  cudaStream_t st = static_cast<cudaStream_t>(stream);
  bool ok;
  BwdBagsWs w = carve_bwd_bags(p, Ns, nb, aligned, true, workspace, workspace_bytes, &ok);
  if ((rc = check_workspace(w.bytes, ok, workspace, workspace_bytes))) return rc;
  DSMIL_CUDA_OK(cudaMemcpyAsync(w.row_offsets, row_offsets, sizeof(long long) * nb, cudaMemcpyHostToDevice, st));
  dsmil_grads_t g{};
  g.gW1 = gW1; g.gb1 = gb1; g.gW2 = gW2; g.gb2 = gb2;
  const float* dz1;
  return bwd_bags_phase3_impl(p, nb, total, Q, H1, dL_local, dqm_global, q_max, crit_idx, w.row_offsets, &g, w, &dz1,
                              st);
}


static int check_bags_dev(const dsmil_params_t* p, bool need_scores, const float* const* Xs, const int64_t* Ns, int nb,
                          int64_t max_rows, const int32_t* status) {
  int rc = check_params(p, need_scores);
  if (rc) return rc;
  DSMIL_REQUIRE(dsmil_shard_bags_supported(p),
                "shape not supported by the batched tensor-core path (D=%d, C=%d, nonlinear=%d, passing_v=%d)", p->D,
                p->C, p->nonlinear, p->passing_v);
  DSMIL_REQUIRE(Xs && Ns && status, "NULL bag list or status");
  DSMIL_REQUIRE(nb >= 1 && nb <= 65535, "nb=%d outside [1, 65535]", nb);
  DSMIL_REQUIRE(max_rows >= 1 && max_rows < 0xffffffffll &&
                static_cast<int64_t>(nb) * ((max_rows + sm90::kTileM - 1) / sm90::kTileM) <= INT_MAX,
                "max_rows=%lld out of range for nb=%d", (long long)max_rows, nb);
  return 0;
}

static BagsWs carve_bags_dev(const dsmil_params_t* p, int nb, int64_t max_rows, void* ws, size_t cap, bool* ok,
                             BagsPlan** plan, float** zero_row) {
  const std::vector<int64_t> Ns(nb, max_rows);
  BagsWs w = carve_bags(p, Ns.data(), nb, false, false, ws, cap, ok);
  Carver c(ws, cap);
  c.off = w.bytes;
  *plan = c.take<BagsPlan>(1);
  *zero_row = c.take<float>(p->D);
  w.bytes = c.off;
  *ok = c.ok();
  return w;
}

size_t dsmil_forward_bags_train_dev_workspace_bytes(const dsmil_params_t* p, int32_t nb, int64_t max_rows) {
  if (!dsmil_shard_bags_supported(p) || nb < 1 || nb > 65535 || max_rows < 1 || max_rows >= 0xffffffffll) return 0;
  bool ok;
  BagsPlan* plan;
  float* zero_row;
  const size_t dev = carve_bags_dev(p, nb, max_rows, nullptr, 0, &ok, &plan, &zero_row).bytes;
  const std::vector<int64_t> Ns(nb, max_rows);
  return std::max(dev, dsmil_forward_bags_train_workspace_bytes(p, Ns.data(), nb));
}

int dsmil_forward_bags_train_dev(const dsmil_params_t* p, const float* const* Xs_dev, const int64_t* Ns_dev,
                                 int32_t nb, int64_t max_rows, float* classes, float* pred, float* A, float* B,
                                 int64_t* crit_idx, float* save_Q, float* save_H1, int32_t* status, void* workspace,
                                 size_t workspace_bytes, void* stream) {
  int rc = check_bags_dev(p, true, Xs_dev, Ns_dev, nb, max_rows, status);
  if (rc) return rc;
  DSMIL_REQUIRE(classes && pred && A && B && crit_idx && save_Q && save_H1, "NULL output pointer");
  const size_t need = dsmil_forward_bags_train_dev_workspace_bytes(p, nb, max_rows);
  if ((rc = check_workspace(need, workspace_bytes >= need, workspace, workspace ? workspace_bytes : 0))) return rc;
  cudaStream_t st = static_cast<cudaStream_t>(stream);
  bool ok;
  BagsPlan* plan;
  float* zero_row;
  BagsWs w = carve_bags_dev(p, nb, max_rows, workspace, workspace_bytes, &ok, &plan, &zero_row);
  k_plan_bags<<<1, 32, 0, st>>>(Xs_dev, Ns_dev, nb, max_rows, p->C, p->D, zero_row, w.table, nullptr, nullptr, plan,
                                status);
  DSMIL_LAUNCH_OK("k_plan_bags");
  DSMIL_CUDA_OK(cudaMemsetAsync(w.keys, 0, sizeof(unsigned long long) * (kMaxC + 1) * nb, st));
  if ((rc = sm90::launch_prep_wimg(p, w.wimg, st))) return rc;
  if ((rc = sm90::launch_qmlp(p, w.table, nb, nb * tiles_for_bag(max_rows), classes, w.keys, save_Q, save_H1, w.wimg,
                              num_sms(), st, false, &plan->tiles)))
    return rc;
  return bags_attend_finalize(p, w, nb, save_Q, false, pred, A, B, crit_idx, nb * recs_for_bag(max_rows), &plan->recs,
                              st);
}

size_t dsmil_backward_bags_dev_workspace_bytes(const dsmil_params_t* p, int32_t nb, int64_t max_rows) {
  if (!dsmil_shard_bags_supported(p) || nb < 1 || nb > 65535 || max_rows < 1 || max_rows >= 0xffffffffll) return 0;
  bool ok;
  return carve_bwd_bags_dev(p, nb, max_rows, nullptr, 0, &ok).bytes;
}

int dsmil_backward_bags_dev(const dsmil_params_t* p, const float* const* Xs_dev, const int64_t* Ns_dev, int32_t nb,
                            int64_t max_rows, const float* Q, const float* H1, const float* A, const float* B,
                            const int64_t* crit_idx, const float* d_classes, const float* d_pred, const float* d_A,
                            const float* d_B, const dsmil_grads_t* grads, int32_t* status, void* workspace,
                            size_t workspace_bytes, void* stream) {
  int rc = check_bags_dev(p, false, Xs_dev, Ns_dev, nb, max_rows, status);
  if (rc) return rc;
  DSMIL_REQUIRE(Q && H1 && A && B && crit_idx && grads, "NULL pointer");
  DSMIL_REQUIRE(!d_A && !d_B && !grads->gX,
                "the dev backward takes gradients through classes and pred only (no d_A, d_B or gX)");
  const size_t need = dsmil_backward_bags_dev_workspace_bytes(p, nb, max_rows);
  if ((rc = check_workspace(need, workspace_bytes >= need, workspace, workspace ? workspace_bytes : 0))) return rc;
  cudaStream_t st = static_cast<cudaStream_t>(stream);
  bool ok;
  BwdBagsWs w = carve_bwd_bags_dev(p, nb, max_rows, workspace, workspace_bytes, &ok);
  k_plan_bags<<<1, 32, 0, st>>>(Xs_dev, Ns_dev, nb, max_rows, p->C, p->D, w.zero_row, w.table, w.chi, w.ch1, w.plan,
                                status);
  DSMIL_LAUNCH_OK("k_plan_bags");
  return backward_bags_run(p, nullptr, nullptr, nb, static_cast<int64_t>(nb) * max_rows, Q, H1, A, B, crit_idx,
                           d_classes, d_pred, nullptr, nullptr, grads, w, st);
}

}
```

dsmil_wsi_b200/csrc/fwd_batched.cuh:

```cuda
#pragma once
#include "common.cuh"
#include "fwd_kernels.cuh"
#include "fwd_sm90.cuh"

namespace dsmil {
namespace sm90 {

constexpr int kAttRows = 128;
constexpr int kMaxRecPerBag = 128;

struct AttendArgs {
  const BagDev* bags;
  int nb;
  int D, C;
  const float* Q;
  bool q_blocked;
  const unsigned long long* keys;
  float* A;
  float* recs;
  const float* qmax_ext;
  const int* nrec_dev;
};

template <int CT, int NJ>
__global__ void __launch_bounds__(256, (NJ == 1 && CT <= 2) ? 5 : 0)
k_attend_b(const AttendArgs a) {
  extern __shared__ __align__(16) float s_dyn[];
  __shared__ __align__(16) float sq[CT][kQ];
  __shared__ float sL[kAttRows][CT];
  __shared__ float sE[kAttRows][CT];
  __shared__ float s_red[8][CT];
  const int tid = threadIdx.x, lane = tid & 31, warp = tid >> 5;
  const int C = a.C, D = a.D;
  if (a.nrec_dev != nullptr && static_cast<int>(blockIdx.x) >= *a.nrec_dev) return;
  const int rec = blockIdx.x;
  int bag = 0;
  while (bag < a.nb - 1 && rec >= a.bags[bag + 1].rec_off) ++bag;
  const BagDev bg = a.bags[bag];
  const int cta_in_bag = rec - bg.rec_off;
  const int ntiles = static_cast<int>((bg.N + kAttRows - 1) / kAttRows);

  for (int i = tid; i < CT * kQ; i += 256) {
    const int k = i / kQ, j = i % kQ;
    float v = 0.f;
    if (k < C && a.qmax_ext != nullptr) {
      v = a.qmax_ext[(static_cast<size_t>(bag) * C + k) * kQ + j];
    } else if (k < C) {
      const long long row = key_row(a.keys[static_cast<size_t>(bag) * kMaxC + k]);
      v = a.q_blocked ? tanh_ex2(a.Q[static_cast<size_t>(bg.tile_off + row / kAttRows) * (kAttRows * kQ) + j * kAttRows + (row % kAttRows)])
                      : a.Q[(bg.row_off + row) * kQ + j];
    }
    sq[k][j] = v;
  }
  float run_m[CT], run_s[CT];
#pragma unroll
  for (int k = 0; k < CT; ++k) { run_m[k] = -INFINITY; run_s[k] = 0.f; }
  float acc[CT][NJ][4];
#pragma unroll
  for (int k = 0; k < CT; ++k)
#pragma unroll
    for (int j = 0; j < NJ; ++j)
#pragma unroll
      for (int e = 0; e < 4; ++e) acc[k][j][e] = 0.f;
  __syncthreads();

  const int half = tid >> 7, c4 = tid & 127;
  const int D4 = D >> 2;
  for (int t = cta_in_bag; t < ntiles; t += bg.nrec) {
    const long long r0 = static_cast<long long>(t) * kAttRows;
    const int rows = static_cast<int>((bg.N - r0) < kAttRows ? (bg.N - r0) : kAttRows);
    float Lr[CT];
#pragma unroll
    for (int k = 0; k < CT; ++k) Lr[k] = -INFINITY;
    if (a.q_blocked) {
      const int r = tid & 127, hf = tid >> 7;
      const float* qb = a.Q + static_cast<size_t>(bg.tile_off + t) * (kAttRows * kQ) + static_cast<size_t>(hf * 64) * kAttRows + r;
      float d[CT];
#pragma unroll
      for (int k = 0; k < CT; ++k) d[k] = 0.f;
#pragma unroll 4
      for (int c = 0; c < 64; c += 4) {
        const float* qc = qb + c * kAttRows;
        const f2 ta = fast_tanh2(f2{__ldg(qc), __ldg(qc + kAttRows)});
        const f2 tb = fast_tanh2(f2{__ldg(qc + 2 * kAttRows), __ldg(qc + 3 * kAttRows)});
#pragma unroll
        for (int k = 0; k < CT; ++k) {
          const float4 w = *reinterpret_cast<const float4*>(&sq[k][hf * 64 + c]);
          d[k] = fmaf(ta.x, w.x, d[k]); d[k] = fmaf(ta.y, w.y, d[k]); d[k] = fmaf(tb.x, w.z, d[k]); d[k] = fmaf(tb.y, w.w, d[k]);
        }
      }
      if (hf == 1) {
#pragma unroll
        for (int k = 0; k < CT; ++k) sE[r][k] = d[k];
      }
      __syncthreads();
      if (hf == 0 && r < rows) {
#pragma unroll
        for (int k = 0; k < CT; ++k) {
          Lr[k] = __fdiv_rn(d[k] + sE[r][k], kScale);
          if (k < C) a.A[(bg.row_off + r0 + r) * C + k] = Lr[k];
        }
      }
    } else {
#pragma unroll 4
      for (int rr = 0; rr < 16; ++rr) {
        const int r = warp * 16 + rr;
        if (r < rows) {
          const float4 q = __ldg(reinterpret_cast<const float4*>(a.Q + (bg.row_off + r0 + r) * kQ) + lane);
#pragma unroll
          for (int k = 0; k < CT; ++k) {
            const float4 w = *reinterpret_cast<const float4*>(&sq[k][lane * 4]);
            float d = q.x * w.x;
            d = fmaf(q.y, w.y, d);
            d = fmaf(q.z, w.z, d);
            d = fmaf(q.w, w.w, d);
            d = warp_sum(d);
            if (lane == 0) {
              const float L = __fdiv_rn(d, kScale);
              sL[r][k] = L;
              if (k < C) a.A[(bg.row_off + r0 + r) * C + k] = L;
            }
          }
        }
      }
      __syncthreads();
      if (tid < rows) {
#pragma unroll
        for (int k = 0; k < CT; ++k) Lr[k] = sL[tid][k];
      }
    }
#pragma unroll
    for (int k = 0; k < CT; ++k) {
      const float v = warp_max(Lr[k]);
      if (lane == 0) s_red[warp][k] = v;
    }
    __syncthreads();
    float mnew[CT], scl[CT], ev[CT];
#pragma unroll
    for (int k = 0; k < CT; ++k) {
      float mx = fmaxf(fmaxf(s_red[0][k], s_red[1][k]), fmaxf(s_red[2][k], s_red[3][k]));
      mnew[k] = fmaxf(run_m[k], mx);
      scl[k] = (run_m[k] == -INFINITY) ? 0.f : expf(run_m[k] - mnew[k]);
      ev[k] = (Lr[k] == -INFINITY) ? 0.f : expf(Lr[k] - mnew[k]);
      if (tid < kAttRows) sE[tid][k] = ev[k];
    }
    __syncthreads();
#pragma unroll
    for (int k = 0; k < CT; ++k) {
      const float v = warp_sum(ev[k]);
      if (lane == 0) s_red[warp][k] = v;
    }
    __syncthreads();
#pragma unroll
    for (int k = 0; k < CT; ++k) {
      run_s[k] = run_s[k] * scl[k] + ((s_red[0][k] + s_red[1][k]) + (s_red[2][k] + s_red[3][k]));
      run_m[k] = mnew[k];
    }
#pragma unroll
    for (int k = 0; k < CT; ++k) {
#pragma unroll
      for (int j = 0; j < NJ; ++j)
#pragma unroll
        for (int e = 0; e < 4; ++e) acc[k][j][e] *= scl[k];
    }
    const float* xb = bg.X + r0 * D;
#pragma unroll 8
    for (int r = half; r < rows; r += 2) {
      float4 x[NJ];
#pragma unroll
      for (int j = 0; j < NJ; ++j) {
        const int col = c4 + 128 * j;
        x[j] = col < D4 ? ldg_stream(reinterpret_cast<const float4*>(xb + static_cast<long long>(r) * D) + col)
                        : make_float4(0.f, 0.f, 0.f, 0.f);
      }
#pragma unroll
      for (int k = 0; k < CT; ++k) {
        const float e = sE[r][k];
#pragma unroll
        for (int j = 0; j < NJ; ++j) {
          acc[k][j][0] = fmaf(e, x[j].x, acc[k][j][0]);
          acc[k][j][1] = fmaf(e, x[j].y, acc[k][j][1]);
          acc[k][j][2] = fmaf(e, x[j].z, acc[k][j][2]);
          acc[k][j][3] = fmaf(e, x[j].w, acc[k][j][3]);
        }
      }
    }
    __syncthreads();
  }
  float* recp = a.recs + static_cast<size_t>(rec) * rec_floats(C, D);
  if (half == 1) {
#pragma unroll
    for (int k = 0; k < CT; ++k)
      if (k < C)
#pragma unroll
        for (int j = 0; j < NJ; ++j) {
          const int col = c4 + 128 * j;
          if (col < D4)
            *reinterpret_cast<float4*>(s_dyn + k * D + col * 4) =
                make_float4(acc[k][j][0], acc[k][j][1], acc[k][j][2], acc[k][j][3]);
        }
  }
  __syncthreads();
  if (half == 0) {
#pragma unroll
    for (int k = 0; k < CT; ++k)
      if (k < C)
#pragma unroll
        for (int j = 0; j < NJ; ++j) {
          const int col = c4 + 128 * j;
          if (col < D4) {
            const float4 o = *reinterpret_cast<const float4*>(s_dyn + k * D + col * 4);
            float* dst = recp + 2 * C + static_cast<size_t>(k) * D + col * 4;
            dst[0] = acc[k][j][0] + o.x;
            dst[1] = acc[k][j][1] + o.y;
            dst[2] = acc[k][j][2] + o.z;
            dst[3] = acc[k][j][3] + o.w;
          }
        }
  }
  if (tid == 0) {
#pragma unroll
    for (int k = 0; k < CT; ++k)
      if (k < C) { recp[k] = run_m[k]; recp[C + k] = run_s[k]; }
  }
}

struct FinalizeArgs {
  const BagDev* bags;
  int D, C;
  const float* recs;
  const unsigned long long* keys;
  const float* Wf;
  const float* bf;
  float* A;
  float* B;
  float* pred;
  long long* crit;
  float* pred_part;
  unsigned int* counters;
  float* emit;
  int ext_P, ext_nb;
};

constexpr int kFinSlices = 32;

__global__ void __launch_bounds__(256, 4)
k_finalize_b(const FinalizeArgs a) {
  __shared__ float sw[kMaxRecPerBag][kMaxC];
  __shared__ float sM[kMaxC], sS[kMaxC];
  __shared__ float s_part[8][32];
  __shared__ float red[kMaxC];
  __shared__ unsigned int s_last;
  const int tid = threadIdx.x, lane = tid & 31, warp = tid >> 5;
  const int C = a.C, D = a.D;
  const int bag = blockIdx.y;
  const BagDev bg = a.bags[bag];
  const size_t rstride = rec_floats(C, D);
  const bool ext = a.ext_P > 0;
  const float* recs = ext ? a.recs + static_cast<size_t>(bag) * rstride : a.recs + static_cast<size_t>(bg.rec_off) * rstride;
  const size_t pstride = ext ? rstride * a.ext_nb : rstride;
  const int P = ext ? a.ext_P : bg.nrec;
  for (int k = warp; k < C; k += 8) {
    float m = -INFINITY;
    for (int p = lane; p < P; p += 32) m = fmaxf(m, recs[p * pstride + k]);
    m = warp_max(m);
    float sacc = 0.f;
    for (int p = lane; p < P; p += 32) {
      const float mp = recs[p * pstride + k];
      const float w = (mp == -INFINITY) ? 0.f : expf(mp - m);
      sw[p][k] = w;
      sacc = fmaf(recs[p * pstride + C + k], w, sacc);
    }
    sacc = warp_sum(sacc);
    if (lane == 0) { sM[k] = m; sS[k] = sacc; }
  }
  __syncthreads();
  if (a.emit == nullptr) {
    const long long total = bg.N * C;
    const long long per = (total + gridDim.x - 1) / gridDim.x;
    const long long lo = per * blockIdx.x, hi = (lo + per) < total ? (lo + per) : total;
    float* Ab = a.A + bg.row_off * C;
    for (long long i = lo + tid; i < hi; i += 256) {
      const int k = static_cast<int>(i % C);
      Ab[i] = __fdiv_rn(expf(Ab[i] - sM[k]), sS[k]);
    }
  }
  const int CD = C * D;
  const int eps = (CD + kFinSlices - 1) / kFinSlices;
  const int e_lo = eps * blockIdx.x, e_hi = (e_lo + eps) < CD ? (e_lo + eps) : CD;
  const int rp = tid >> 5;
  float ppart[kMaxC];
#pragma unroll
  for (int k = 0; k < kMaxC; ++k) ppart[k] = 0.f;
  for (int base = e_lo; base < e_hi; base += 32) {
    const int e = base + lane;
    float acc = 0.f;
    if (e < e_hi) {
      const int k = e / D;
      const float* col = recs + 2 * C + e;
#pragma unroll 1
      for (int p0 = rp; p0 < P; p0 += 64) {
        float v[8];
#pragma unroll
        for (int u = 0; u < 8; ++u) v[u] = (p0 + 8 * u < P) ? col[static_cast<size_t>(p0 + 8 * u) * pstride] : 0.f;
#pragma unroll
        for (int u = 0; u < 8; ++u)
          if (p0 + 8 * u < P) acc = fmaf(v[u], sw[p0 + 8 * u][k], acc);
      }
    }
    s_part[rp][lane] = acc;
    __syncthreads();
    if (rp == 0 && e < e_hi) {
      float tot = s_part[0][lane];
#pragma unroll
      for (int r = 1; r < 8; ++r) tot += s_part[r][lane];
      if (a.emit != nullptr) {
        a.emit[static_cast<size_t>(bag) * rstride + 2 * C + e] = tot;
      } else {
        const int k = e / D;
        const float bval = __fdiv_rn(tot, sS[k]);
        a.B[static_cast<size_t>(bag) * CD + e] = bval;
        for (int kk = 0; kk < C; ++kk) ppart[kk] = fmaf(__ldg(a.Wf + static_cast<size_t>(kk) * CD + e), bval, ppart[kk]);
      }
    }
    __syncthreads();
  }
  if (a.emit != nullptr) {
    if (blockIdx.x == 0 && tid < C) {
      a.emit[static_cast<size_t>(bag) * rstride + tid] = sM[tid];
      a.emit[static_cast<size_t>(bag) * rstride + C + tid] = sS[tid];
    }
    return;
  }
  if (warp == 0) {
    for (int kk = 0; kk < C; ++kk) {
      const float v = warp_sum(ppart[kk]);
      if (lane == 0) red[kk] = v;
    }
  }
  __syncthreads();
  float* part = a.pred_part + (static_cast<size_t>(bag) * kFinSlices + blockIdx.x) * kMaxC;
  if (tid < C) part[tid] = red[tid];
  __threadfence();
  __syncthreads();
  if (tid == 0) s_last = atomicAdd(a.counters + bag, 1u);
  __syncthreads();
  if (s_last != kFinSlices - 1) return;
  __threadfence();
  if (tid < C) {
    const volatile float* pp = a.pred_part + static_cast<size_t>(bag) * kFinSlices * kMaxC;
    float sacc = 0.f;
    for (int sl = 0; sl < kFinSlices; ++sl) sacc += pp[sl * kMaxC + tid];
    a.pred[static_cast<size_t>(bag) * C + tid] = sacc + __ldg(a.bf + tid);
    if (a.crit) a.crit[static_cast<size_t>(bag) * C + tid] = key_row(a.keys[static_cast<size_t>(bag) * kMaxC + tid]);
  }
}

__global__ void __launch_bounds__(128)
k_gather_cand_b(const BagDev* __restrict__ bags, const unsigned long long* __restrict__ keys,
                const float* __restrict__ classes, const float* __restrict__ Q, bool q_blocked,
                const long long* __restrict__ row_offsets, int C, float* __restrict__ cands) {
  const int k = blockIdx.x, bag = blockIdx.y;
  const BagDev bg = bags[bag];
  float* cand = cands + static_cast<size_t>(bag) * cand_floats(C);
  long long* idx = reinterpret_cast<long long*>(cand);
  float* score = cand + 2 * C;
  float* qrow = cand + 3 * C + static_cast<size_t>(k) * kQ;
  const unsigned long long key = keys[static_cast<size_t>(bag) * kMaxC + k];
  if (bg.N <= 0 || key == 0ull) {
    if (threadIdx.x == 0) { idx[k] = INT64_MAX; score[k] = -INFINITY; }
    qrow[threadIdx.x] = 0.f;
    return;
  }
  const long long row = key_row(key);
  if (threadIdx.x == 0) {
    idx[k] = row + row_offsets[bag];
    score[k] = classes[(bg.row_off + row) * C + k];
  }
  qrow[threadIdx.x] = q_blocked
      ? tanh_ex2(Q[static_cast<size_t>(bg.tile_off + row / kAttRows) * (kAttRows * kQ) + threadIdx.x * kAttRows + (row % kAttRows)])
      : Q[(bg.row_off + row) * kQ + threadIdx.x];
}

inline bool batched_supported(const dsmil_params_t* p) {
  return qmlp_supported(p) && !p->passing_v && p->D % 4 == 0 && p->D <= 2048 && p->C <= 4 &&
         ((p->C <= 2) || p->D <= 1024);
}

inline int launch_attend_b(const AttendArgs& a, int nrecs, cudaStream_t st) {
  const int C = a.C, D = a.D;
  const size_t smem = sizeof(float) * C * D;
  const int NJ = D <= 512 ? 1 : (D <= 1024 ? 2 : 4);
  auto go = [&](auto kern) -> int {
    if (smem > 48 * 1024)
      DSMIL_CUDA_OK(cudaFuncSetAttribute(kern, cudaFuncAttributeMaxDynamicSharedMemorySize, static_cast<int>(smem)));
    prof_begin(PROF_ATTEND, st);
    kern<<<nrecs, 256, smem, st>>>(a);
    prof_end(PROF_ATTEND, st);
    DSMIL_LAUNCH_OK("k_attend_b");
    return 0;
  };
  if (C == 1) { if (NJ == 1) return go(k_attend_b<1, 1>); if (NJ == 2) return go(k_attend_b<1, 2>); return go(k_attend_b<1, 4>); }
  if (C == 2) { if (NJ == 1) return go(k_attend_b<2, 1>); if (NJ == 2) return go(k_attend_b<2, 2>); return go(k_attend_b<2, 4>); }
  if (NJ == 1) return go(k_attend_b<4, 1>);
  return go(k_attend_b<4, 2>);
}

inline int launch_finalize_b(const FinalizeArgs& a, int nb, cudaStream_t st) {
  prof_begin(PROF_FINAL, st);
  k_finalize_b<<<dim3(kFinSlices, nb), 256, 0, st>>>(a);
  prof_end(PROF_FINAL, st);
  DSMIL_LAUNCH_OK("k_finalize_b");
  return 0;
}

}
}
```

dsmil_wsi_b200/csrc/fwd_sm90.cuh:

```cuda
#pragma once
#include <cuda_bf16.h>
#include <cstdlib>

#include "common.cuh"

namespace dsmil {
namespace sm90 {

constexpr int kTileM = 128;
constexpr int kChunkK = 64;
constexpr int kTileBytes = kQ * kChunkK * 2;
constexpr int kChunkBytes = 2 * kTileBytes;
constexpr int kWStages = 4;
constexpr int kPrefetchChunks = 2;
constexpr int kConsumerWGs = 2;
constexpr int kWarpProd = 4 * kConsumerWGs;
constexpr int kThreads = 128 * (kConsumerWGs + 1);
constexpr int kRegsConsumer = 232, kRegsProducer = 40;
template <int R> __device__ __forceinline__ void reg_inc() { asm volatile("setmaxnreg.inc.sync.aligned.u32 %0;" ::"n"(R)); }
template <int R> __device__ __forceinline__ void reg_dec() { asm volatile("setmaxnreg.dec.sync.aligned.u32 %0;" ::"n"(R)); }

__device__ __forceinline__ float4 lds128(uint32_t addr) {
  float4 v;
  asm volatile("ld.shared.v4.f32 {%0,%1,%2,%3}, [%4];" : "=f"(v.x), "=f"(v.y), "=f"(v.z), "=f"(v.w) : "r"(addr));
  return v;
}
__device__ __forceinline__ float4 ldg_stream(const float4* p) {
  float4 v;
  asm volatile("ld.global.nc.L1::no_allocate.v4.f32 {%0,%1,%2,%3}, [%4];"
               : "=f"(v.x), "=f"(v.y), "=f"(v.z), "=f"(v.w) : "l"(p));
  return v;
}
__device__ __forceinline__ void prefetch_l2(const void* p) { asm volatile("prefetch.global.L2 [%0];" ::"l"(p)); }

__device__ __forceinline__ uint32_t smem_u32(const void* p) { return static_cast<uint32_t>(__cvta_generic_to_shared(p)); }
__device__ __forceinline__ void mbar_init(uint32_t bar, uint32_t count) {
  asm volatile("mbarrier.init.shared::cta.b64 [%0], %1;" ::"r"(bar), "r"(count));
}
__device__ __forceinline__ void mbar_arrive(uint32_t bar) {
  asm volatile("mbarrier.arrive.shared::cta.b64 _, [%0];" ::"r"(bar) : "memory");
}
__device__ __forceinline__ void mbar_expect_tx(uint32_t bar, uint32_t bytes) {
  asm volatile("mbarrier.arrive.expect_tx.shared::cta.b64 _, [%0], %1;" ::"r"(bar), "r"(bytes) : "memory");
}
__device__ __forceinline__ void mbar_wait(uint32_t bar, uint32_t parity, uint32_t sleep_ns = 0) {
  uint32_t done = 0, spins = 0;
  while (true) {
    asm volatile(
        "{\n\t.reg .pred p;\n\t"
        "mbarrier.try_wait.parity.shared::cta.b64 p, [%1], %2;\n\t"
        "selp.u32 %0, 1, 0, p;\n\t}"
        : "=r"(done) : "r"(bar), "r"(parity) : "memory");
    if (done) break;
    if (sleep_ns) __nanosleep(sleep_ns);
    if (++spins > (1u << 26)) __trap();
  }
}
__device__ __forceinline__ void bulk_g2s(uint32_t dst, const void* src, uint32_t bytes, uint32_t bar) {
  asm volatile("cp.async.bulk.shared::cluster.global.mbarrier::complete_tx::bytes [%0], [%1], %2, [%3];"
               ::"r"(dst), "l"(src), "r"(bytes), "r"(bar) : "memory");
}

__device__ __forceinline__ uint64_t smem_desc(uint32_t saddr) {
  return static_cast<uint64_t>(((saddr & 0x3ffffu) >> 4) | (1u << 16)) |
         (static_cast<uint64_t>((1024u >> 4) | (1u << 30)) << 32);
}
__device__ __forceinline__ void wg_fence() { asm volatile("wgmma.fence.sync.aligned;" ::: "memory"); }
__device__ __forceinline__ void wg_commit() { asm volatile("wgmma.commit_group.sync.aligned;" ::: "memory"); }
__device__ __forceinline__ void wg_wait0() { asm volatile("wgmma.wait_group.sync.aligned 0;" ::: "memory"); }
__device__ __forceinline__ void fence_acc(float (&d)[64]) {
#pragma unroll
  for (int i = 0; i < 64; ++i) asm volatile("" : "+f"(d[i])::"memory");
}
__device__ __forceinline__ void mma_rs(float (&d)[64], uint32_t a0, uint32_t a1, uint32_t a2, uint32_t a3, uint64_t b,
                                       uint32_t acc) {
  asm volatile(
      "{\n\t.reg .pred p;\n\tsetp.ne.b32 p, %68, 0;\n\t"
      "wgmma.mma_async.sync.aligned.m64n128k16.f32.bf16.bf16 "
      "{%0, %1, %2, %3, %4, %5, %6, %7, %8, %9, %10, %11, %12, %13, %14, %15, %16, %17, %18, %19, %20, %21, %22, %23, "
      "%24, %25, %26, %27, %28, %29, %30, %31, %32, %33, %34, %35, %36, %37, %38, %39, %40, %41, %42, %43, %44, %45, "
      "%46, %47, %48, %49, %50, %51, %52, %53, %54, %55, %56, %57, %58, %59, %60, %61, %62, %63}, "
      "{%64, %65, %66, %67}, %69, p, 1, 1, 0;\n\t}"
      : "+f"(d[0]), "+f"(d[1]), "+f"(d[2]), "+f"(d[3]), "+f"(d[4]), "+f"(d[5]), "+f"(d[6]), "+f"(d[7]), "+f"(d[8]),
        "+f"(d[9]), "+f"(d[10]), "+f"(d[11]), "+f"(d[12]), "+f"(d[13]), "+f"(d[14]), "+f"(d[15]), "+f"(d[16]),
        "+f"(d[17]), "+f"(d[18]), "+f"(d[19]), "+f"(d[20]), "+f"(d[21]), "+f"(d[22]), "+f"(d[23]), "+f"(d[24]),
        "+f"(d[25]), "+f"(d[26]), "+f"(d[27]), "+f"(d[28]), "+f"(d[29]), "+f"(d[30]), "+f"(d[31]), "+f"(d[32]),
        "+f"(d[33]), "+f"(d[34]), "+f"(d[35]), "+f"(d[36]), "+f"(d[37]), "+f"(d[38]), "+f"(d[39]), "+f"(d[40]),
        "+f"(d[41]), "+f"(d[42]), "+f"(d[43]), "+f"(d[44]), "+f"(d[45]), "+f"(d[46]), "+f"(d[47]), "+f"(d[48]),
        "+f"(d[49]), "+f"(d[50]), "+f"(d[51]), "+f"(d[52]), "+f"(d[53]), "+f"(d[54]), "+f"(d[55]), "+f"(d[56]),
        "+f"(d[57]), "+f"(d[58]), "+f"(d[59]), "+f"(d[60]), "+f"(d[61]), "+f"(d[62]), "+f"(d[63])
      : "r"(a0), "r"(a1), "r"(a2), "r"(a3), "r"(acc), "l"(b));
}

__host__ __device__ inline uint32_t swz_off(int row, int k) {
  return static_cast<uint32_t>(row * 128 + ((((k >> 3) ^ (row & 7)) & 7) << 4) + ((k & 7) << 1));
}
__host__ __device__ inline int kLogicalK(int p) {
  const int q = (p & 15) >> 2, t = p & 3;
  return (p & ~15) + (t < 2 ? 2 * q + t : 8 + 2 * q + t - 2);
}

struct BagDev {
  const float* X;
  long long N;
  long long row_off;
  int tile_off;
  int rec_off;
  int nrec;
  int pad_;
};

constexpr int kSmemBags = 96;

struct QmlpArgs {
  const BagDev* bags;
  int nb, ntiles;
  int D, C;
  const float* Wi;
  const float* bi;
  const float* b1;
  const float* b2;
  const uint8_t* w1img;
  const uint8_t* w2img;
  float* classes;
  unsigned long long* keys;
  float* Q;
  float* H1;
  bool q_blocked;
  const int* ntiles_dev;
};

struct TileCursor {
  const BagDev* bags;
  int bag, last;
  __device__ TileCursor(const BagDev* b, int nb) : bags(b), bag(0), last(nb - 1) {}
  __device__ __forceinline__ void seek(int tile) {
    while (bag < last && tile >= bags[bag + 1].tile_off) ++bag;
  }
};

struct f2 { float x, y; };
__device__ __forceinline__ float tanh_ex2(float x) {
  const float t = __fmul_rn(x, 2.8853900817779268f);
  float e, r;
  asm("ex2.approx.ftz.f32 %0, %1;" : "=f"(e) : "f"(t));
  asm("rcp.approx.ftz.f32 %0, %1;" : "=f"(r) : "f"(__fadd_rn(e, 1.f)));
  return __fmaf_rn(r, -2.f, 1.f);
}
__device__ __forceinline__ f2 fast_tanh2(f2 x) { return f2{tanh_ex2(x.x), tanh_ex2(x.y)}; }

constexpr int kOffWRing = 0;
constexpr int kOffWi = kOffWRing + kWStages * kChunkBytes;
constexpr int kSmemFixed = kOffWi;

template <int CT, int DT, bool DEV = false>
__global__ void __launch_bounds__(kThreads, 1)
k_qmlp_sm90(const QmlpArgs a) {
  extern __shared__ uint8_t smem_raw[];
  uint8_t* smem = reinterpret_cast<uint8_t*>((reinterpret_cast<uintptr_t>(smem_raw) + 1023) & ~uintptr_t(1023));
  __shared__ __align__(8) uint64_t bars[2 * kWStages];
  __shared__ __align__(16) float s_b1[kQ], s_b2[kQ];
  __shared__ BagDev s_bags[kSmemBags];

  const int tid = threadIdx.x, warp = tid >> 5, lane = tid & 31;
  const int D = DT ? DT : a.D, C = a.C;
  const int nchunks = D / kChunkK;
  auto live = [&](int t) { return t < a.ntiles && (!DEV || t < *a.ntiles_dev); };
  enum { W_FULL = 0, W_EMPTY = kWStages };
  auto bar = [&](int i) { return smem_u32(&bars[i]); };

  float* sWi = reinterpret_cast<float*>(smem + kOffWi);
  const bool do_scores = a.classes != nullptr;
  if (do_scores)
    for (int i = tid; i < CT * D; i += kThreads) sWi[i] = (i < C * D) ? a.Wi[i] : 0.f;
  if (tid < kQ) { s_b1[tid] = a.b1[tid]; s_b2[tid] = a.b2[tid]; }
  const bool tbl_in_smem = a.nb <= kSmemBags;
  if (tbl_in_smem)
    for (int i = tid; i < a.nb; i += kThreads) s_bags[i] = a.bags[i];
  const BagDev* tbl = tbl_in_smem ? s_bags : a.bags;
  if (tid == 0) {
    for (int s = 0; s < kWStages; ++s) { mbar_init(bar(W_FULL + s), 1); mbar_init(bar(W_EMPTY + s), kConsumerWGs); }
    asm volatile("fence.mbarrier_init.release.cluster;" ::: "memory");
  }
  __syncthreads();

  if (warp >= kWarpProd) {
    reg_dec<kRegsProducer>();
    if (warp == kWarpProd && lane == 0) {
      uint32_t stage = 0, phase = 0;
      auto push = [&](const uint8_t* src) {
        mbar_wait(bar(W_EMPTY + stage), phase ^ 1, 256);
        mbar_expect_tx(bar(W_FULL + stage), kChunkBytes);
        bulk_g2s(smem_u32(smem + kOffWRing + stage * kChunkBytes), src, kChunkBytes, bar(W_FULL + stage));
        if (++stage == kWStages) { stage = 0; phase ^= 1; }
      };
      for (int tile = blockIdx.x; live(tile); tile += gridDim.x) {
        for (int kc = 0; kc < nchunks; ++kc) push(a.w1img + static_cast<size_t>(kc) * kChunkBytes);
        push(a.w2img);
        push(a.w2img + kChunkBytes);
      }
    }
    return;
  }

  reg_inc<kRegsConsumer>();
  const int q = lane & 3;
  const int rloc = (warp >> 2) * 64 + (warp & 3) * 16 + (lane >> 2);
  const uint32_t swi_u32 = smem_u32(sWi) + 16u * q;
  const uint32_t wring = smem_u32(smem + kOffWRing);
  const bool signaller = (warp & 3) == 0 && lane == 0;
  uint32_t ws = 0, wph = 0;
  auto w_next = [&]() -> uint32_t {
    const uint32_t s = ws;
    mbar_wait(bar(W_FULL + s), wph);
    if (++ws == kWStages) { ws = 0; wph ^= 1; }
    return s;
  };
  auto w_release = [&](uint32_t s) {
    if (signaller) mbar_arrive(bar(W_EMPTY + s));
  };

  TileCursor cur_bag(tbl, a.nb);
  uint32_t ld_N = 0, ld_row = 0;
  bool ld_full = false;
  long long ld_rowoff = 0;
  const float* xrow = nullptr;
  auto open_tile = [&](int t) {
    cur_bag.seek(t);
    const BagDev* bp = tbl + cur_bag.bag;
    ld_N = static_cast<uint32_t>(bp->N);
    ld_rowoff = bp->row_off;
    ld_row = static_cast<uint32_t>(t - bp->tile_off) * kTileM + rloc;
    ld_full = ld_row - rloc + kTileM <= ld_N;
    xrow = bp->X + static_cast<long long>(ld_row) * D + 4 * q;
  };
  auto load_chunk = [&](int kc, float4 (&x)[8]) {
    if ((CT <= 4 || DT != 0) && kc + kPrefetchChunks < nchunks && (ld_full || ld_row + 8 * (q >> 1) < ld_N))
      prefetch_l2(xrow - 4 * q + static_cast<long long>(q >> 1) * (8ll * D) + (kc + kPrefetchChunks) * kChunkK + (q & 1) * 32);
#pragma unroll
    for (int s = 0; s < 4; ++s)
#pragma unroll
      for (int i = 0; i < 2; ++i) {
        const float4* src = reinterpret_cast<const float4*>(xrow + static_cast<long long>(i) * (8ll * D) + kc * kChunkK + 16 * s);
        x[2 * s + i] = (ld_full || ld_row + 8 * i < ld_N) ? ldg_stream(src) : make_float4(0.f, 0.f, 0.f, 0.f);
      }
  };
  float sc[2][CT];
  auto convert = [&](const float4 (&x)[8], int kc, uint32_t (&hi)[16], uint32_t (&lo)[16]) {
#pragma unroll
    for (int s = 0; s < 4; ++s) {
      if (do_scores) {
#pragma unroll
        for (int k = 0; k < CT; ++k) {
          const float4 w = lds128(swi_u32 + static_cast<uint32_t>(k * D + kc * kChunkK + 16 * s) * 4u);
#pragma unroll
          for (int i = 0; i < 2; ++i) {
            const float4 v = x[2 * s + i];
            float t = sc[i][k];
            t = fmaf(v.x, w.x, t); t = fmaf(v.y, w.y, t); t = fmaf(v.z, w.z, t); t = fmaf(v.w, w.w, t);
            sc[i][k] = t;
          }
        }
      }
#pragma unroll
      for (int i = 0; i < 2; ++i) {
        const float4 v = x[2 * s + i];
        const __nv_bfloat162 h01 = __floats2bfloat162_rn(v.x, v.y), h23 = __floats2bfloat162_rn(v.z, v.w);
        const uint32_t u01 = *reinterpret_cast<const uint32_t*>(&h01), u23 = *reinterpret_cast<const uint32_t*>(&h23);
        const __nv_bfloat162 l01 = __floats2bfloat162_rn(v.x - __uint_as_float(u01 << 16), v.y - __uint_as_float(u01 & 0xffff0000u));
        const __nv_bfloat162 l23 = __floats2bfloat162_rn(v.z - __uint_as_float(u23 << 16), v.w - __uint_as_float(u23 & 0xffff0000u));
        hi[4 * s + i] = u01;
        hi[4 * s + 2 + i] = u23;
        lo[4 * s + i] = *reinterpret_cast<const uint32_t*>(&l01);
        lo[4 * s + 2 + i] = *reinterpret_cast<const uint32_t*>(&l23);
      }
    }
  };
  float acc[64];
  auto mma_chunk = [&](const uint32_t (&hi)[16], const uint32_t (&lo)[16], int kc) -> uint32_t {
    const uint32_t st = w_next();
    const uint64_t bh = smem_desc(wring + st * kChunkBytes), bl = bh + (kTileBytes >> 4);
    wg_fence();
#pragma unroll
    for (int s = 0; s < 4; ++s) {
      mma_rs(acc, hi[4 * s], hi[4 * s + 1], hi[4 * s + 2], hi[4 * s + 3], bh + 2 * s, (kc | s) != 0);
      mma_rs(acc, lo[4 * s], lo[4 * s + 1], lo[4 * s + 2], lo[4 * s + 3], bh + 2 * s, 1);
      mma_rs(acc, hi[4 * s], hi[4 * s + 1], hi[4 * s + 2], hi[4 * s + 3], bl + 2 * s, 1);
    }
    wg_commit();
    return st;
  };

  int tile = blockIdx.x;
  float4 x[8];
  if (live(tile)) { open_tile(tile); load_chunk(0, x); }
  uint32_t ha[16], la[16], hb[16], lb[16];
  while (live(tile)) {
    const int my_bag = cur_bag.bag;
    const uint32_t t_N = ld_N, t_row = ld_row;
    const long long t_rowoff = ld_rowoff;
    const int next_tile = tile + gridDim.x;
#pragma unroll
    for (int i = 0; i < 2; ++i)
#pragma unroll
      for (int k = 0; k < CT; ++k) sc[i][k] = 0.f;
#pragma unroll
    for (int i = 0; i < 64; ++i) acc[i] = 0.f;
    convert(x, 0, ha, la);
    load_chunk(1, x);
#pragma unroll 1
    for (int kc = 0; kc < nchunks; kc += 2) {
      const uint32_t s0 = mma_chunk(ha, la, kc);
      convert(x, kc + 1, hb, lb);
      if (kc + 2 < nchunks) load_chunk(kc + 2, x);
      else if (live(next_tile)) { open_tile(next_tile); load_chunk(0, x); }
      wg_wait0();
      fence_acc(acc);
      w_release(s0);
      const uint32_t s1 = mma_chunk(hb, lb, kc + 1);
      if (kc + 2 < nchunks) { convert(x, kc + 2, ha, la); load_chunk(kc + 3, x); }
      wg_wait0();
      fence_acc(acc);
      w_release(s1);
    }
    if (do_scores) {
      unsigned long long best[CT];
#pragma unroll
      for (int k = 0; k < CT; ++k) best[k] = 0ull;
#pragma unroll
      for (int i = 0; i < 2; ++i) {
        const uint32_t n = t_row + 8 * i;
#pragma unroll
        for (int k = 0; k < CT; ++k) {
          float v = sc[i][k];
          v += __shfl_xor_sync(0xffffffffu, v, 2);
          v += __shfl_xor_sync(0xffffffffu, v, 1);
          if (q == 0 && k < C && n < t_N) {
            v += a.bi[k];
            a.classes[(t_rowoff + n) * C + k] = v;
            const unsigned long long key = pack_key(v, n);
            best[k] = key > best[k] ? key : best[k];
          }
        }
      }
#pragma unroll
      for (int k = 0; k < CT; ++k) {
        const unsigned long long b = warp_max_u64(best[k]);
        if (lane == 0 && k < C && b) atomicMax(a.keys + static_cast<size_t>(my_bag) * kMaxC + k, b);
      }
    }
    uint32_t h2[32], l2[32];
#pragma unroll
    for (int j = 0; j < 16; ++j) {
      const float2 bb = *reinterpret_cast<const float2*>(&s_b1[8 * j + 2 * q]);
#pragma unroll
      for (int i = 0; i < 2; ++i) {
        const float h0 = fmaxf(acc[4 * j + 2 * i] + bb.x, 0.f), h1 = fmaxf(acc[4 * j + 2 * i + 1] + bb.y, 0.f);
        if (a.H1 != nullptr && t_row + 8 * i < t_N)
          *reinterpret_cast<float2*>(a.H1 + (t_rowoff + t_row + 8 * i) * kQ + 8 * j + 2 * q) = make_float2(h0, h1);
        const __nv_bfloat162 hh = __floats2bfloat162_rn(h0, h1);
        const uint32_t hu = *reinterpret_cast<const uint32_t*>(&hh);
        const __nv_bfloat162 ll = __floats2bfloat162_rn(h0 - __uint_as_float(hu << 16), h1 - __uint_as_float(hu & 0xffff0000u));
        h2[4 * (j >> 1) + 2 * (j & 1) + i] = hu;
        l2[4 * (j >> 1) + 2 * (j & 1) + i] = *reinterpret_cast<const uint32_t*>(&ll);
      }
    }
    float qa[64];
#pragma unroll
    for (int i = 0; i < 64; ++i) qa[i] = 0.f;
    const uint32_t w0 = w_next(), w1 = w_next();
    {
      const uint64_t b0 = smem_desc(wring + w0 * kChunkBytes), b1 = smem_desc(wring + w1 * kChunkBytes);
      wg_fence();
#pragma unroll
      for (int s = 0; s < 8; ++s) {
        const uint64_t bh = (s < 4 ? b0 : b1) + 2 * (s & 3), bl = bh + (kTileBytes >> 4);
        mma_rs(qa, h2[4 * s], h2[4 * s + 1], h2[4 * s + 2], h2[4 * s + 3], bh, s > 0);
        mma_rs(qa, l2[4 * s], l2[4 * s + 1], l2[4 * s + 2], l2[4 * s + 3], bh, 1);
        mma_rs(qa, h2[4 * s], h2[4 * s + 1], h2[4 * s + 2], h2[4 * s + 3], bl, 1);
      }
      wg_commit();
      wg_wait0();
      fence_acc(qa);
      w_release(w0);
      w_release(w1);
    }
#pragma unroll
    for (int j = 0; j < 16; ++j) {
      const int c = 8 * j + 2 * q;
      const float2 bb = *reinterpret_cast<const float2*>(&s_b2[c]);
#pragma unroll
      for (int i = 0; i < 2; ++i) {
        const float z0 = qa[4 * j + 2 * i] + bb.x, z1 = qa[4 * j + 2 * i + 1] + bb.y;
        if (a.q_blocked) {
          float* dst = a.Q + static_cast<size_t>(tile) * (kTileM * kQ) + static_cast<size_t>(c) * kTileM + rloc + 8 * i;
          dst[0] = z0;
          dst[kTileM] = z1;
        } else if (t_row + 8 * i < t_N) {
          *reinterpret_cast<float2*>(a.Q + (t_rowoff + t_row + 8 * i) * kQ + c) = make_float2(tanh_ex2(z0), tanh_ex2(z1));
        }
      }
    }
    tile = next_tile;
  }
}

__global__ void __launch_bounds__(256)
k_prep_wimg2(const float* __restrict__ W1, int D, const float* __restrict__ W2, uint8_t* __restrict__ img1,
             uint8_t* __restrict__ img2) {
  const int t1 = 128 * D, total = t1 + 128 * kQ;
  for (int i = blockIdx.x * blockDim.x + threadIdx.x; i < total; i += gridDim.x * blockDim.x) {
    const bool first = i < t1;
    const int K = first ? D : kQ;
    const int j = first ? i : i - t1;
    const int n = j / K, k = j % K;
    const float w = first ? W1[j] : W2[j];
    const __nv_bfloat16 hi = __float2bfloat16_rn(w);
    const __nv_bfloat16 lo = __float2bfloat16_rn(w - __bfloat162float(hi));
    uint8_t* chunk = (first ? img1 : img2) + static_cast<size_t>(k / kChunkK) * kChunkBytes;
    const uint32_t off = swz_off(n, first ? kLogicalK(k % kChunkK) : k % kChunkK);
    *reinterpret_cast<__nv_bfloat16*>(chunk + off) = hi;
    *reinterpret_cast<__nv_bfloat16*>(chunk + kTileBytes + off) = lo;
  }
}

inline size_t qmlp_smem_bytes(int C, int D) {
  const int ct = C <= 1 ? 1 : (C <= 2 ? 2 : (C <= 4 ? 4 : 8));
  return kSmemFixed + sizeof(float) * ct * D + 1024;
}
inline size_t wimg_bytes(int D) { return static_cast<size_t>(D / kChunkK) * kChunkBytes + 2 * kChunkBytes; }
inline bool qmlp_supported(const dsmil_params_t* p) {
  return p->nonlinear && p->D % (2 * kChunkK) == 0 &&
         qmlp_smem_bytes(p->C, p->D) + 2 * kQ * sizeof(float) + kSmemBags * sizeof(BagDev) + 256 <= 232448;
}

inline int launch_prep_wimg(const dsmil_params_t* p, uint8_t* wimg, cudaStream_t st) {
  uint8_t* w2img = wimg + static_cast<size_t>(p->D / kChunkK) * kChunkBytes;
  k_prep_wimg2<<<80, 256, 0, st>>>(p->W1, p->D, p->W2, wimg, w2img);
  DSMIL_LAUNCH_OK("k_prep_wimg2");
  return 0;
}

inline int launch_qmlp(const dsmil_params_t* p, const BagDev* bags_dev, int nb, int ntiles, float* classes,
                       unsigned long long* keys, float* Q, float* H1, const uint8_t* wimg, int num_sms, cudaStream_t st,
                       bool q_blocked, const int* ntiles_dev = nullptr) {
  const int D = p->D, C = p->C;
  if (ntiles_dev != nullptr && C > 4) {
    set_error("launch_qmlp: a device tile count needs C <= 4");
    return DSMIL_ERR_ARG;
  }
  const uint8_t* w2img = wimg + static_cast<size_t>(D / kChunkK) * kChunkBytes;
  QmlpArgs a{bags_dev, nb, ntiles, D, C, p->Wi, p->bi, p->b1, p->b2, wimg, w2img, classes, keys, Q, H1, q_blocked,
             ntiles_dev};
  const size_t smem = qmlp_smem_bytes(C, D);
  const int grid = ntiles < num_sms ? ntiles : num_sms;
  auto go = [&](auto kern) -> int {
    DSMIL_CUDA_OK(cudaFuncSetAttribute(kern, cudaFuncAttributeMaxDynamicSharedMemorySize, static_cast<int>(smem)));
    prof_begin(PROF_FUSED, st);
    kern<<<grid, kThreads, smem, st>>>(a);
    prof_end(PROF_FUSED, st);
    DSMIL_LAUNCH_OK("k_qmlp_sm90");
    return 0;
  };
  if (ntiles_dev != nullptr) {
    if (D == 512) {
      if (C == 1) return go(k_qmlp_sm90<1, 512, true>);
      if (C == 2) return go(k_qmlp_sm90<2, 512, true>);
      return go(k_qmlp_sm90<4, 512, true>);
    }
    if (C == 1) return go(k_qmlp_sm90<1, 0, true>);
    if (C == 2) return go(k_qmlp_sm90<2, 0, true>);
    return go(k_qmlp_sm90<4, 0, true>);
  }
  if (D == 512) {
    if (C == 1) return go(k_qmlp_sm90<1, 512>);
    if (C == 2) return go(k_qmlp_sm90<2, 512>);
    if (C <= 4) return go(k_qmlp_sm90<4, 512>);
    return go(k_qmlp_sm90<8, 512>);
  }
  if (C == 1) return go(k_qmlp_sm90<1, 0>);
  if (C == 2) return go(k_qmlp_sm90<2, 0>);
  if (C <= 4) return go(k_qmlp_sm90<4, 0>);
  return go(k_qmlp_sm90<8, 0>);
}

}
}
```

Measured before the change: 386.5 million.

## Fuse attention pass into persistent QMLP kernel via cooperative launch and per-bag counters

Moves the attention/record stage into the persistent sm90 QMLP kernel. Each CTA, once its bag's Q tiles are all written (tracked by atomic per-bag done counters and a spin-wait), runs attend_record on a work unit, optionally preloading its Q tile. This drops a separate kernel launch and the gap between the Q write and the attention read, and Q is read through L2 while it is still hot. In exchange it needs a cooperative launch for forward progress, more shared memory per CTA, and a spin-wait that can stall CTAs when bags finish unevenly.

```diff
diff --git a/dsmil_wsi_b200/csrc/abi.cu b/dsmil_wsi_b200/csrc/abi.cu
--- a/dsmil_wsi_b200/csrc/abi.cu
+++ b/dsmil_wsi_b200/csrc/abi.cu
@@ -177,7 +177,8 @@
 
 static int bags_phase1_impl(const dsmil_params_t* p, const Phase1Ws& w, const float* const* Xs, const int64_t* Ns,
                             int nb, const float* classes_in, float* classes, float* Q, float* H1, bool q_blocked,
-                            bool upload, int* tiles, int* recs, cudaStream_t st) {
+                            bool upload, int* tiles, int* recs, cudaStream_t st,
+                            const sm90::AttendFuse* fuse = nullptr) {
   std::vector<sm90::BagDev> tbl;
   int rc;
   if ((rc = build_table(Xs, Ns, nb, tbl, tiles, recs))) return rc;
@@ -190,6 +191,9 @@
     k_argmax<<<grid, 256, 0, st>>>(classes_in, Ns[0], p->C, w.keys);
     DSMIL_LAUNCH_OK("k_argmax");
   }
+  if (fuse)
+    return sm90::launch_qmlp_attend(p, w.table, nb, *tiles, classes_in ? nullptr : classes, w.keys, Q, w.wimg,
+                                    w.counters + nb, *fuse, st);
   return sm90::launch_qmlp(p, w.table, nb, *tiles, classes_in ? nullptr : classes, w.keys, Q, H1, w.wimg, num_sms(),
                            st, q_blocked);
 }
@@ -406,16 +410,19 @@
   return w;
 }
 
+static int bags_finalize(const dsmil_params_t* p, const BagsWs& w, int nb, float* pred, float* A, float* B,
+                         int64_t* crit, cudaStream_t st) {
+  sm90::FinalizeArgs fa{w.table, p->D, p->C, w.recs, w.keys, p->Wf, p->bf, A, B, pred,
+                         reinterpret_cast<long long*>(crit), w.pred_part, w.counters, nullptr, 0, 0};
+  return sm90::launch_finalize_b(fa, nb, st);
+}
 static int bags_attend_finalize(const dsmil_params_t* p, const BagsWs& w, int nb, const float* Q, bool q_blocked,
                                 float* pred, float* A, float* B, int64_t* crit, int recs, const int* recs_dev,
                                 cudaStream_t st) {
-  const int C = p->C, D = p->D;
   int rc;
-  sm90::AttendArgs aa{w.table, nb, D, C, Q, q_blocked, w.keys, A, w.recs, nullptr, recs_dev};
+  sm90::AttendArgs aa{w.table, nb, p->D, p->C, Q, q_blocked, w.keys, A, w.recs, nullptr, recs_dev};
   if ((rc = sm90::launch_attend_b(aa, recs, st))) return rc;
-  sm90::FinalizeArgs fa{w.table, D, C, w.recs, w.keys, p->Wf, p->bf, A, B, pred, reinterpret_cast<long long*>(crit),
-                         w.pred_part, w.counters, nullptr, 0, 0};
-  return sm90::launch_finalize_b(fa, nb, st);
+  return bags_finalize(p, w, nb, pred, A, B, crit, st);
 }
 
 static int forward_bags_impl(const dsmil_params_t* p, const float* const* Xs, const int64_t* Ns, int nb,
@@ -429,8 +436,12 @@
   float* Q = save_Q ? save_Q : w.Q;
   const bool q_blocked = save_Q == nullptr;
   int tiles, recs;
-  if ((rc = bags_phase1_impl(p, w, Xs, Ns, nb, classes_in, classes, Q, save_H1, q_blocked, true, &tiles, &recs, st)))
+  sm90::AttendFuse fuse{A, w.recs, 0, 0};
+  const bool fused = q_blocked && save_H1 == nullptr && sm90::plan_attend_fuse(p, Ns, nb, num_sms(), &fuse);
+  if ((rc = bags_phase1_impl(p, w, Xs, Ns, nb, classes_in, classes, Q, save_H1, q_blocked, true, &tiles, &recs, st,
+                             fused ? &fuse : nullptr)))
     return rc;
+  if (fused) return bags_finalize(p, w, nb, pred, A, B, crit, st);
   return bags_attend_finalize(p, w, nb, Q, q_blocked, pred, A, B, crit, recs, nullptr, st);
 }
 
diff --git a/dsmil_wsi_b200/csrc/fwd_batched.cuh b/dsmil_wsi_b200/csrc/fwd_batched.cuh
--- a/dsmil_wsi_b200/csrc/fwd_batched.cuh
+++ b/dsmil_wsi_b200/csrc/fwd_batched.cuh
@@ -5,22 +5,6 @@
 
 namespace dsmil {
 namespace sm90 {
-
-constexpr int kAttRows = 128;
-constexpr int kMaxRecPerBag = 128;
-
-struct AttendArgs {
-  const BagDev* bags;
-  int nb;
-  int D, C;
-  const float* Q;
-  bool q_blocked;
-  const unsigned long long* keys;
-  float* A;
-  float* recs;
-  const float* qmax_ext;
-  const int* nrec_dev;
-};
 
 template <int CT, int NJ>
 __global__ void __launch_bounds__(256, (NJ == 1 && CT <= 2) ? 5 : 0)
@@ -30,199 +14,12 @@
   __shared__ float sL[kAttRows][CT];
   __shared__ float sE[kAttRows][CT];
   __shared__ float s_red[8][CT];
-  const int tid = threadIdx.x, lane = tid & 31, warp = tid >> 5;
-  const int C = a.C, D = a.D;
   if (a.nrec_dev != nullptr && static_cast<int>(blockIdx.x) >= *a.nrec_dev) return;
   const int rec = blockIdx.x;
   int bag = 0;
   while (bag < a.nb - 1 && rec >= a.bags[bag + 1].rec_off) ++bag;
   const BagDev bg = a.bags[bag];
-  const int cta_in_bag = rec - bg.rec_off;
-  const int ntiles = static_cast<int>((bg.N + kAttRows - 1) / kAttRows);
-
-  for (int i = tid; i < CT * kQ; i += 256) {
-    const int k = i / kQ, j = i % kQ;
-    float v = 0.f;
-    if (k < C && a.qmax_ext != nullptr) {
-      v = a.qmax_ext[(static_cast<size_t>(bag) * C + k) * kQ + j];
-    } else if (k < C) {
-      const long long row = key_row(a.keys[static_cast<size_t>(bag) * kMaxC + k]);
-      v = a.q_blocked ? tanh_ex2(a.Q[static_cast<size_t>(bg.tile_off + row / kAttRows) * (kAttRows * kQ) + j * kAttRows + (row % kAttRows)])
-                      : a.Q[(bg.row_off + row) * kQ + j];
-    }
-    sq[k][j] = v;
-  }
-  float run_m[CT], run_s[CT];
-#pragma unroll
-  for (int k = 0; k < CT; ++k) { run_m[k] = -INFINITY; run_s[k] = 0.f; }
-  float acc[CT][NJ][4];
-#pragma unroll
-  for (int k = 0; k < CT; ++k)
-#pragma unroll
-    for (int j = 0; j < NJ; ++j)
-#pragma unroll
-      for (int e = 0; e < 4; ++e) acc[k][j][e] = 0.f;
-  __syncthreads();
-
-  const int half = tid >> 7, c4 = tid & 127;
-  const int D4 = D >> 2;
-  for (int t = cta_in_bag; t < ntiles; t += bg.nrec) {
-    const long long r0 = static_cast<long long>(t) * kAttRows;
-    const int rows = static_cast<int>((bg.N - r0) < kAttRows ? (bg.N - r0) : kAttRows);
-    float Lr[CT];
-#pragma unroll
-    for (int k = 0; k < CT; ++k) Lr[k] = -INFINITY;
-    if (a.q_blocked) {
-      const int r = tid & 127, hf = tid >> 7;
-      const float* qb = a.Q + static_cast<size_t>(bg.tile_off + t) * (kAttRows * kQ) + static_cast<size_t>(hf * 64) * kAttRows + r;
-      float d[CT];
-#pragma unroll
-      for (int k = 0; k < CT; ++k) d[k] = 0.f;
-#pragma unroll 4
-      for (int c = 0; c < 64; c += 4) {
-        const float* qc = qb + c * kAttRows;
-        const f2 ta = fast_tanh2(f2{__ldg(qc), __ldg(qc + kAttRows)});
-        const f2 tb = fast_tanh2(f2{__ldg(qc + 2 * kAttRows), __ldg(qc + 3 * kAttRows)});
-#pragma unroll
-        for (int k = 0; k < CT; ++k) {
-          const float4 w = *reinterpret_cast<const float4*>(&sq[k][hf * 64 + c]);
-          d[k] = fmaf(ta.x, w.x, d[k]); d[k] = fmaf(ta.y, w.y, d[k]); d[k] = fmaf(tb.x, w.z, d[k]); d[k] = fmaf(tb.y, w.w, d[k]);
-        }
-      }
-      if (hf == 1) {
-#pragma unroll
-        for (int k = 0; k < CT; ++k) sE[r][k] = d[k];
-      }
-      __syncthreads();
-      if (hf == 0 && r < rows) {
-#pragma unroll
-        for (int k = 0; k < CT; ++k) {
-          Lr[k] = __fdiv_rn(d[k] + sE[r][k], kScale);
-          if (k < C) a.A[(bg.row_off + r0 + r) * C + k] = Lr[k];
-        }
-      }
-    } else {
-#pragma unroll 4
-      for (int rr = 0; rr < 16; ++rr) {
-        const int r = warp * 16 + rr;
-        if (r < rows) {
-          const float4 q = __ldg(reinterpret_cast<const float4*>(a.Q + (bg.row_off + r0 + r) * kQ) + lane);
-#pragma unroll
-          for (int k = 0; k < CT; ++k) {
-            const float4 w = *reinterpret_cast<const float4*>(&sq[k][lane * 4]);
-            float d = q.x * w.x;
-            d = fmaf(q.y, w.y, d);
-            d = fmaf(q.z, w.z, d);
-            d = fmaf(q.w, w.w, d);
-            d = warp_sum(d);
-            if (lane == 0) {
-              const float L = __fdiv_rn(d, kScale);
-              sL[r][k] = L;
-              if (k < C) a.A[(bg.row_off + r0 + r) * C + k] = L;
-            }
-          }
-        }
-      }
-      __syncthreads();
-      if (tid < rows) {
-#pragma unroll
-        for (int k = 0; k < CT; ++k) Lr[k] = sL[tid][k];
-      }
-    }
-#pragma unroll
-    for (int k = 0; k < CT; ++k) {
-      const float v = warp_max(Lr[k]);
-      if (lane == 0) s_red[warp][k] = v;
-    }
-    __syncthreads();
-    float mnew[CT], scl[CT], ev[CT];
-#pragma unroll
-    for (int k = 0; k < CT; ++k) {
-      float mx = fmaxf(fmaxf(s_red[0][k], s_red[1][k]), fmaxf(s_red[2][k], s_red[3][k]));
-      mnew[k] = fmaxf(run_m[k], mx);
-      scl[k] = (run_m[k] == -INFINITY) ? 0.f : expf(run_m[k] - mnew[k]);
-      ev[k] = (Lr[k] == -INFINITY) ? 0.f : expf(Lr[k] - mnew[k]);
-      if (tid < kAttRows) sE[tid][k] = ev[k];
-    }
-    __syncthreads();
-#pragma unroll
-    for (int k = 0; k < CT; ++k) {
-      const float v = warp_sum(ev[k]);
-      if (lane == 0) s_red[warp][k] = v;
-    }
-    __syncthreads();
-#pragma unroll
-    for (int k = 0; k < CT; ++k) {
-      run_s[k] = run_s[k] * scl[k] + ((s_red[0][k] + s_red[1][k]) + (s_red[2][k] + s_red[3][k]));
-      run_m[k] = mnew[k];
-    }
-#pragma unroll
-    for (int k = 0; k < CT; ++k) {
-#pragma unroll
-      for (int j = 0; j < NJ; ++j)
-#pragma unroll
-        for (int e = 0; e < 4; ++e) acc[k][j][e] *= scl[k];
-    }
-    const float* xb = bg.X + r0 * D;
-#pragma unroll 8
-    for (int r = half; r < rows; r += 2) {
-      float4 x[NJ];
-#pragma unroll
-      for (int j = 0; j < NJ; ++j) {
-        const int col = c4 + 128 * j;
-        x[j] = col < D4 ? ldg_stream(reinterpret_cast<const float4*>(xb + static_cast<long long>(r) * D) + col)
-                        : make_float4(0.f, 0.f, 0.f, 0.f);
-      }
-#pragma unroll
-      for (int k = 0; k < CT; ++k) {
-        const float e = sE[r][k];
-#pragma unroll
-        for (int j = 0; j < NJ; ++j) {
-          acc[k][j][0] = fmaf(e, x[j].x, acc[k][j][0]);
-          acc[k][j][1] = fmaf(e, x[j].y, acc[k][j][1]);
-          acc[k][j][2] = fmaf(e, x[j].z, acc[k][j][2]);
-          acc[k][j][3] = fmaf(e, x[j].w, acc[k][j][3]);
-        }
-      }
-    }
-    __syncthreads();
-  }
-  float* recp = a.recs + static_cast<size_t>(rec) * rec_floats(C, D);
-  if (half == 1) {
-#pragma unroll
-    for (int k = 0; k < CT; ++k)
-      if (k < C)
-#pragma unroll
-        for (int j = 0; j < NJ; ++j) {
-          const int col = c4 + 128 * j;
-          if (col < D4)
-            *reinterpret_cast<float4*>(s_dyn + k * D + col * 4) =
-                make_float4(acc[k][j][0], acc[k][j][1], acc[k][j][2], acc[k][j][3]);
-        }
-  }
-  __syncthreads();
-  if (half == 0) {
-#pragma unroll
-    for (int k = 0; k < CT; ++k)
-      if (k < C)
-#pragma unroll
-        for (int j = 0; j < NJ; ++j) {
-          const int col = c4 + 128 * j;
-          if (col < D4) {
-            const float4 o = *reinterpret_cast<const float4*>(s_dyn + k * D + col * 4);
-            float* dst = recp + 2 * C + static_cast<size_t>(k) * D + col * 4;
-            dst[0] = acc[k][j][0] + o.x;
-            dst[1] = acc[k][j][1] + o.y;
-            dst[2] = acc[k][j][2] + o.z;
-            dst[3] = acc[k][j][3] + o.w;
-          }
-        }
-  }
-  if (tid == 0) {
-#pragma unroll
-    for (int k = 0; k < CT; ++k)
-      if (k < C) { recp[k] = run_m[k]; recp[C + k] = run_s[k]; }
-  }
+  attend_record<CT, NJ, CtaSync, false>(a, bag, bg, rec, s_dyn, sq, sL, sE, s_red);
 }
 
 struct FinalizeArgs {
@@ -406,6 +203,74 @@
   return go(k_attend_b<4, 2>);
 }
 
+inline size_t qmlp_attend_smem_bytes(int C, int D) {
+  const int ct = C <= 1 ? 1 : (C <= 2 ? 2 : 4);
+  return qmlp_smem_bytes(C, D) + sizeof(float) * (static_cast<size_t>(ct) * (kQ + 2 * kAttRows + 8) + static_cast<size_t>(C) * D);
+}
+
+struct AttendFuse {
+  float* A;
+  float* recs;
+  int nunits, grid;
+};
+
+template <int CT, int DT>
+inline auto qmlp_attend_kernel() { return k_qmlp_sm90<CT, DT, false, true>; }
+inline auto qmlp_attend_kernel(int C, int D) {
+  if (D == 512) return C == 1 ? qmlp_attend_kernel<1, 512>() : (C == 2 ? qmlp_attend_kernel<2, 512>() : qmlp_attend_kernel<4, 512>());
+  return C == 1 ? qmlp_attend_kernel<1, 0>() : (C == 2 ? qmlp_attend_kernel<2, 0>() : qmlp_attend_kernel<4, 0>());
+}
+
+inline bool plan_attend_fuse(const dsmil_params_t* p, const int64_t* Ns, int nb, int num_sms, AttendFuse* f) {
+  if (!batched_supported(p)) return false;
+  for (int b = 0; b < nb; ++b)
+    if (Ns[b] > static_cast<int64_t>(kAttRows) * kMaxRecPerBag) return false;
+  const size_t smem = qmlp_attend_smem_bytes(p->C, p->D);
+  if (smem + 2 * kQ * sizeof(float) + kSmemBags * sizeof(BagDev) + 256 > 232448) return false;
+  int dev = 0, coop = 0, occ = 0;
+  if (cudaGetDevice(&dev) != cudaSuccess || cudaDeviceGetAttribute(&coop, cudaDevAttrCooperativeLaunch, dev) != cudaSuccess ||
+      !coop)
+    return false;
+  auto kern = qmlp_attend_kernel(p->C, p->D);
+  if (cudaFuncSetAttribute(kern, cudaFuncAttributeMaxDynamicSharedMemorySize, static_cast<int>(smem)) != cudaSuccess ||
+      cudaOccupancyMaxActiveBlocksPerMultiprocessor(&occ, kern, kThreads, smem) != cudaSuccess) {
+    cudaGetLastError();
+    return false;
+  }
+  f->nunits = attend_units(Ns, nb);
+  f->grid = f->nunits < num_sms ? f->nunits : num_sms;
+  return occ >= 1 && f->grid <= occ * num_sms;
+}
+
+inline int launch_qmlp_attend(const dsmil_params_t* p, const BagDev* bags_dev, int nb, int ntiles, float* classes,
+                              unsigned long long* keys, float* Q, const uint8_t* wimg, unsigned int* done,
+                              const AttendFuse& f, cudaStream_t st) {
+  const int D = p->D, C = p->C;
+  const uint8_t* w2img = wimg + static_cast<size_t>(D / kChunkK) * kChunkBytes;
+  const QmlpArgs a{bags_dev, nb, ntiles, D, C, p->Wi, p->bi, p->b1, p->b2, wimg, w2img, classes, keys, Q, nullptr, true,
+                   nullptr};
+  const AttendOut att{f.A, f.recs, done, f.nunits};
+  const size_t smem = qmlp_attend_smem_bytes(C, D);
+  auto kern = qmlp_attend_kernel(C, D);
+  DSMIL_CUDA_OK(cudaFuncSetAttribute(kern, cudaFuncAttributeMaxDynamicSharedMemorySize, static_cast<int>(smem)));
+  cudaLaunchAttribute attr[1];
+  attr[0].id = cudaLaunchAttributeCooperative;
+  attr[0].val.cooperative = 1;
+  cudaLaunchConfig_t cfg = {};
+  cfg.gridDim = dim3(f.grid);
+  cfg.blockDim = dim3(kThreads);
+  cfg.dynamicSmemBytes = smem;
+  cfg.stream = st;
+  cfg.attrs = attr;
+  cfg.numAttrs = 1;
+  prof_begin(PROF_FUSED, st);
+  const cudaError_t e = cudaLaunchKernelEx(&cfg, kern, a, att);
+  prof_end(PROF_FUSED, st);
+  DSMIL_CUDA_OK(e);
+  DSMIL_LAUNCH_OK("k_qmlp_sm90 (attend)");
+  return 0;
+}
+
 inline int launch_finalize_b(const FinalizeArgs& a, int nb, cudaStream_t st) {
   prof_begin(PROF_FINAL, st);
   k_finalize_b<<<dim3(kFinSlices, nb), 256, 0, st>>>(a);
diff --git a/dsmil_wsi_b200/csrc/fwd_sm90.cuh b/dsmil_wsi_b200/csrc/fwd_sm90.cuh
--- a/dsmil_wsi_b200/csrc/fwd_sm90.cuh
+++ b/dsmil_wsi_b200/csrc/fwd_sm90.cuh
@@ -3,6 +3,7 @@
 #include <cstdlib>
 
 #include "common.cuh"
+#include "fwd_kernels.cuh"
 
 namespace dsmil {
 namespace sm90 {
@@ -129,6 +130,12 @@
   bool q_blocked;
   const int* ntiles_dev;
 };
+struct AttendOut {
+  float* A;
+  float* recs;
+  unsigned int* done;
+  int nunits;
+};
 
 struct TileCursor {
   const BagDev* bags;
@@ -149,13 +156,284 @@
 }
 __device__ __forceinline__ f2 fast_tanh2(f2 x) { return f2{tanh_ex2(x.x), tanh_ex2(x.y)}; }
 
+constexpr int kAttRows = 128;
+constexpr int kMaxRecPerBag = 128;
+
+struct AttendArgs {
+  const BagDev* bags;
+  int nb;
+  int D, C;
+  const float* Q;
+  bool q_blocked;
+  const unsigned long long* keys;
+  float* A;
+  float* recs;
+  const float* qmax_ext;
+  const int* nrec_dev;
+};
+
+struct CtaSync { __device__ __forceinline__ static void sync() { __syncthreads(); } };
+struct ConsumerSync { __device__ __forceinline__ static void sync() { asm volatile("bar.sync 1, 256;" ::: "memory"); } };
+
+template <int CT, int NJ, class Sync, bool COHERENT, bool PRELOAD = false>
+__device__ __forceinline__ void attend_record(const AttendArgs& a, int bag, const BagDev& bg, int rec, float* s_dyn,
+                                              float (*sq)[kQ], float (*sL)[CT], float (*sE)[CT], float (*s_red)[CT]) {
+  const int tid = threadIdx.x, lane = tid & 31, warp = tid >> 5;
+  const int C = a.C, D = a.D;
+  const int cta_in_bag = rec - bg.rec_off;
+  const int ntiles = static_cast<int>((bg.N + kAttRows - 1) / kAttRows);
+  float qpre[PRELOAD ? 64 : 1];
+  if constexpr (PRELOAD) {
+    const float* qb = a.Q + static_cast<size_t>(bg.tile_off + cta_in_bag) * (kAttRows * kQ) +
+                      static_cast<size_t>((tid >> 7) * 64) * kAttRows + (tid & 127);
+#pragma unroll
+    for (int c = 0; c < 64; ++c) qpre[c] = COHERENT ? __ldcg(qb + c * kAttRows) : __ldg(qb + c * kAttRows);
+  }
+
+  for (int i = tid; i < CT * kQ; i += 256) {
+    const int k = i / kQ, j = i % kQ;
+    float v = 0.f;
+    if (k < C && a.qmax_ext != nullptr) {
+      v = a.qmax_ext[(static_cast<size_t>(bag) * C + k) * kQ + j];
+    } else if (k < C) {
+      const unsigned long long* kp = a.keys + static_cast<size_t>(bag) * kMaxC + k;
+      const long long row = key_row(COHERENT ? __ldcg(kp) : *kp);
+      const float* qb = a.Q + static_cast<size_t>(bg.tile_off + row / kAttRows) * (kAttRows * kQ) + j * kAttRows + (row % kAttRows);
+      const float* qr = a.Q + (bg.row_off + row) * kQ + j;
+      if (COHERENT) v = a.q_blocked ? tanh_ex2(__ldcg(qb)) : __ldcg(qr);
+      else v = a.q_blocked ? tanh_ex2(*qb) : *qr;
+    }
+    sq[k][j] = v;
+  }
+  float run_m[CT], run_s[CT];
+#pragma unroll
+  for (int k = 0; k < CT; ++k) { run_m[k] = -INFINITY; run_s[k] = 0.f; }
+  float acc[CT][NJ][4];
+#pragma unroll
+  for (int k = 0; k < CT; ++k)
+#pragma unroll
+    for (int j = 0; j < NJ; ++j)
+#pragma unroll
+      for (int e = 0; e < 4; ++e) acc[k][j][e] = 0.f;
+  Sync::sync();
+
+  const int half = tid >> 7, c4 = tid & 127;
+  const int D4 = D >> 2;
+  for (int t = cta_in_bag; t < ntiles; t += bg.nrec) {
+    const long long r0 = static_cast<long long>(t) * kAttRows;
+    const int rows = static_cast<int>((bg.N - r0) < kAttRows ? (bg.N - r0) : kAttRows);
+    float Lr[CT];
+#pragma unroll
+    for (int k = 0; k < CT; ++k) Lr[k] = -INFINITY;
+    if (a.q_blocked) {
+      const int r = tid & 127, hf = tid >> 7;
+      const float* qb = a.Q + static_cast<size_t>(bg.tile_off + t) * (kAttRows * kQ) + static_cast<size_t>(hf * 64) * kAttRows + r;
+      float d[CT];
+#pragma unroll
+      for (int k = 0; k < CT; ++k) d[k] = 0.f;
+#pragma unroll (PRELOAD ? 16 : 4)
+      for (int c = 0; c < 64; c += 4) {
+        const float* qc = qb + c * kAttRows;
+        f2 ta, tb;
+        if constexpr (PRELOAD) {
+          ta = fast_tanh2(f2{qpre[c], qpre[c + 1]});
+          tb = fast_tanh2(f2{qpre[c + 2], qpre[c + 3]});
+        } else {
+          ta = COHERENT ? fast_tanh2(f2{__ldcg(qc), __ldcg(qc + kAttRows)})
+                        : fast_tanh2(f2{__ldg(qc), __ldg(qc + kAttRows)});
+          tb = COHERENT ? fast_tanh2(f2{__ldcg(qc + 2 * kAttRows), __ldcg(qc + 3 * kAttRows)})
+                        : fast_tanh2(f2{__ldg(qc + 2 * kAttRows), __ldg(qc + 3 * kAttRows)});
+        }
+#pragma unroll
+        for (int k = 0; k < CT; ++k) {
+          const float4 w = *reinterpret_cast<const float4*>(&sq[k][hf * 64 + c]);
+          d[k] = fmaf(ta.x, w.x, d[k]); d[k] = fmaf(ta.y, w.y, d[k]); d[k] = fmaf(tb.x, w.z, d[k]); d[k] = fmaf(tb.y, w.w, d[k]);
+        }
+      }
+      if (hf == 1) {
+#pragma unroll
+        for (int k = 0; k < CT; ++k) sE[r][k] = d[k];
+      }
+      Sync::sync();
+      if (hf == 0 && r < rows) {
+#pragma unroll
+        for (int k = 0; k < CT; ++k) {
+          Lr[k] = __fdiv_rn(d[k] + sE[r][k], kScale);
+          if (k < C) a.A[(bg.row_off + r0 + r) * C + k] = Lr[k];
+        }
+      }
+    } else {
+#pragma unroll 4
+      for (int rr = 0; rr < 16; ++rr) {
+        const int r = warp * 16 + rr;
+        if (r < rows) {
+          const float4* qp = reinterpret_cast<const float4*>(a.Q + (bg.row_off + r0 + r) * kQ) + lane;
+          const float4 q = COHERENT ? __ldcg(qp) : __ldg(qp);
+#pragma unroll
+          for (int k = 0; k < CT; ++k) {
+            const float4 w = *reinterpret_cast<const float4*>(&sq[k][lane * 4]);
+            float d = q.x * w.x;
+            d = fmaf(q.y, w.y, d);
+            d = fmaf(q.z, w.z, d);
+            d = fmaf(q.w, w.w, d);
+            d = warp_sum(d);
+            if (lane == 0) {
+              const float L = __fdiv_rn(d, kScale);
+              sL[r][k] = L;
+              if (k < C) a.A[(bg.row_off + r0 + r) * C + k] = L;
+            }
+          }
+        }
+      }
+      Sync::sync();
+      if (tid < rows) {
+#pragma unroll
+        for (int k = 0; k < CT; ++k) Lr[k] = sL[tid][k];
+      }
+    }
+#pragma unroll
+    for (int k = 0; k < CT; ++k) {
+      const float v = warp_max(Lr[k]);
+      if (lane == 0) s_red[warp][k] = v;
+    }
+    Sync::sync();
+    float mnew[CT], scl[CT], ev[CT];
+#pragma unroll
+    for (int k = 0; k < CT; ++k) {
+      float mx = fmaxf(fmaxf(s_red[0][k], s_red[1][k]), fmaxf(s_red[2][k], s_red[3][k]));
+      mnew[k] = fmaxf(run_m[k], mx);
+      scl[k] = (run_m[k] == -INFINITY) ? 0.f : expf(run_m[k] - mnew[k]);
+      ev[k] = (Lr[k] == -INFINITY) ? 0.f : expf(Lr[k] - mnew[k]);
+      if (tid < kAttRows) sE[tid][k] = ev[k];
+    }
+    Sync::sync();
+#pragma unroll
+    for (int k = 0; k < CT; ++k) {
+      const float v = warp_sum(ev[k]);
+      if (lane == 0) s_red[warp][k] = v;
+    }
+    Sync::sync();
+#pragma unroll
+    for (int k = 0; k < CT; ++k) {
+      run_s[k] = run_s[k] * scl[k] + ((s_red[0][k] + s_red[1][k]) + (s_red[2][k] + s_red[3][k]));
+      run_m[k] = mnew[k];
+    }
+#pragma unroll
+    for (int k = 0; k < CT; ++k) {
+#pragma unroll
+      for (int j = 0; j < NJ; ++j)
+#pragma unroll
+        for (int e = 0; e < 4; ++e) acc[k][j][e] *= scl[k];
+    }
+    const float* xb = bg.X + r0 * D;
+#pragma unroll (PRELOAD && NJ == 1 && CT <= 2 ? 16 : 8)
+    for (int r = half; r < rows; r += 2) {
+      float4 x[NJ];
+#pragma unroll
+      for (int j = 0; j < NJ; ++j) {
+        const int col = c4 + 128 * j;
+        x[j] = col < D4 ? ldg_stream(reinterpret_cast<const float4*>(xb + static_cast<long long>(r) * D) + col)
+                        : make_float4(0.f, 0.f, 0.f, 0.f);
+      }
+#pragma unroll
+      for (int k = 0; k < CT; ++k) {
+        const float e = sE[r][k];
+#pragma unroll
+        for (int j = 0; j < NJ; ++j) {
+          acc[k][j][0] = fmaf(e, x[j].x, acc[k][j][0]);
+          acc[k][j][1] = fmaf(e, x[j].y, acc[k][j][1]);
+          acc[k][j][2] = fmaf(e, x[j].z, acc[k][j][2]);
+          acc[k][j][3] = fmaf(e, x[j].w, acc[k][j][3]);
+        }
+      }
+    }
+    Sync::sync();
+  }
+  float* recp = a.recs + static_cast<size_t>(rec) * rec_floats(C, D);
+  if (half == 1) {
+#pragma unroll
+    for (int k = 0; k < CT; ++k)
+      if (k < C)
+#pragma unroll
+        for (int j = 0; j < NJ; ++j) {
+          const int col = c4 + 128 * j;
+          if (col < D4)
+            *reinterpret_cast<float4*>(s_dyn + k * D + col * 4) =
+                make_float4(acc[k][j][0], acc[k][j][1], acc[k][j][2], acc[k][j][3]);
+        }
+  }
+  Sync::sync();
+  if (half == 0) {
+#pragma unroll
+    for (int k = 0; k < CT; ++k)
+      if (k < C)
+#pragma unroll
+        for (int j = 0; j < NJ; ++j) {
+          const int col = c4 + 128 * j;
+          if (col < D4) {
+            const float4 o = *reinterpret_cast<const float4*>(s_dyn + k * D + col * 4);
+            float* dst = recp + 2 * C + static_cast<size_t>(k) * D + col * 4;
+            dst[0] = acc[k][j][0] + o.x;
+            dst[1] = acc[k][j][1] + o.y;
+            dst[2] = acc[k][j][2] + o.z;
+            dst[3] = acc[k][j][3] + o.w;
+          }
+        }
+  }
+  if (tid == 0) {
+#pragma unroll
+    for (int k = 0; k < CT; ++k)
+      if (k < C) { recp[k] = run_m[k]; recp[C + k] = run_s[k]; }
+  }
+}
+
+struct UnitCursor {
+  const BagDev* bags;
+  int nb, seg, start, len;
+  __device__ UnitCursor(const BagDev* b, int n) : bags(b), nb(n), seg(-1), start(0), len(0) {}
+  __device__ __forceinline__ int tiles(int b) const { return static_cast<int>((bags[b].N + kTileM - 1) / kTileM); }
+  __device__ __forceinline__ int seg_len(int s) const {
+    const int t = s < nb ? tiles(s) : 0, r = s > 0 ? bags[s - 1].nrec : 0;
+    return t > r ? t : r;
+  }
+  __device__ __forceinline__ void seek(int u) {
+    while (u >= start + len) { start += len; len = seg_len(++seg); }
+  }
+  __device__ __forceinline__ int p1_tile(int u) const {
+    return (seg < nb && u - start < tiles(seg)) ? bags[seg].tile_off + (u - start) : -1;
+  }
+  __device__ __forceinline__ int att_pos(int u) const { return (seg > 0 && u - start < bags[seg - 1].nrec) ? u - start : -1; }
+};
+inline int attend_units(const int64_t* Ns, int nb) {
+  int u = 0;
+  for (int s = 0; s <= nb; ++s) {
+    const int t = s < nb ? static_cast<int>((Ns[s] + kTileM - 1) / kTileM) : 0;
+    const int64_t rt = s > 0 ? (Ns[s - 1] + kAttRows - 1) / kAttRows : 0;
+    const int r = static_cast<int>(rt < kMaxRecPerBag ? rt : kMaxRecPerBag);
+    u += t > r ? t : r;
+  }
+  return u;
+}
+
+__device__ __forceinline__ void wait_count(const unsigned int* p, unsigned int target) {
+  uint32_t spins = 0;
+  while (true) {
+    unsigned int v;
+    asm volatile("ld.acquire.gpu.global.u32 %0, [%1];" : "=r"(v) : "l"(p) : "memory");
+    if (v >= target) break;
+    __nanosleep(64);
+    if (++spins > (1u << 26)) __trap();
+  }
+}
+
 constexpr int kOffWRing = 0;
 constexpr int kOffWi = kOffWRing + kWStages * kChunkBytes;
 constexpr int kSmemFixed = kOffWi;
 
-template <int CT, int DT, bool DEV = false>
+template <int CT, int DT, bool DEV = false, bool ATTEND = false>
 __global__ void __launch_bounds__(kThreads, 1)
-k_qmlp_sm90(const QmlpArgs a) {
+k_qmlp_sm90(const QmlpArgs a, const AttendOut att) {
+  static_assert(!(ATTEND && (DEV || CT > 4)), "the ATTEND form is the eager eval form with C <= 4");
   extern __shared__ uint8_t smem_raw[];
   uint8_t* smem = reinterpret_cast<uint8_t*>((reinterpret_cast<uintptr_t>(smem_raw) + 1023) & ~uintptr_t(1023));
   __shared__ __align__(8) uint64_t bars[2 * kWStages];
@@ -194,10 +472,19 @@
         bulk_g2s(smem_u32(smem + kOffWRing + stage * kChunkBytes), src, kChunkBytes, bar(W_FULL + stage));
         if (++stage == kWStages) { stage = 0; phase ^= 1; }
       };
-      for (int tile = blockIdx.x; live(tile); tile += gridDim.x) {
+      auto push_tile = [&]() {
         for (int kc = 0; kc < nchunks; ++kc) push(a.w1img + static_cast<size_t>(kc) * kChunkBytes);
         push(a.w2img);
         push(a.w2img + kChunkBytes);
+      };
+      if constexpr (ATTEND) {
+        UnitCursor uc(tbl, a.nb);
+        for (int u = blockIdx.x; u < att.nunits; u += gridDim.x) {
+          uc.seek(u);
+          if (uc.p1_tile(u) >= 0) push_tile();
+        }
+      } else {
+        for (int tile = blockIdx.x; live(tile); tile += gridDim.x) push_tile();
       }
     }
     return;
@@ -291,117 +578,160 @@
     return st;
   };
 
-  int tile = blockIdx.x;
+  UnitCursor uc(tbl, a.nb), lc(tbl, a.nb);
+  auto next_p1 = [&](int u) -> int {
+    for (; u < att.nunits; u += gridDim.x) {
+      lc.seek(u);
+      const int t = lc.p1_tile(u);
+      if (t >= 0) return t;
+    }
+    return -1;
+  };
+  int unit = blockIdx.x;
+  int tile = ATTEND ? next_p1(unit) : static_cast<int>(blockIdx.x);
   float4 x[8];
-  if (live(tile)) { open_tile(tile); load_chunk(0, x); }
+  if (ATTEND ? tile >= 0 : live(tile)) { open_tile(tile); load_chunk(0, x); }
   uint32_t ha[16], la[16], hb[16], lb[16];
-  while (live(tile)) {
-    const int my_bag = cur_bag.bag;
-    const uint32_t t_N = ld_N, t_row = ld_row;
-    const long long t_rowoff = ld_rowoff;
-    const int next_tile = tile + gridDim.x;
-#pragma unroll
-    for (int i = 0; i < 2; ++i)
-#pragma unroll
-      for (int k = 0; k < CT; ++k) sc[i][k] = 0.f;
-#pragma unroll
-    for (int i = 0; i < 64; ++i) acc[i] = 0.f;
-    convert(x, 0, ha, la);
-    load_chunk(1, x);
+  while (ATTEND ? unit < att.nunits : live(tile)) {
+    bool p1 = true;
+    int rpos = -1, next_tile;
+    if constexpr (ATTEND) {
+      uc.seek(unit);
+      p1 = uc.p1_tile(unit) >= 0;
+      rpos = uc.att_pos(unit);
+      next_tile = p1 ? next_p1(unit + gridDim.x) : tile;
+    } else {
+      next_tile = tile + gridDim.x;
+    }
+    if (p1) {
+      const int my_bag = cur_bag.bag;
+      const uint32_t t_N = ld_N, t_row = ld_row;
+      const long long t_rowoff = ld_rowoff;
+#pragma unroll
+      for (int i = 0; i < 2; ++i)
+#pragma unroll
+        for (int k = 0; k < CT; ++k) sc[i][k] = 0.f;
+#pragma unroll
+      for (int i = 0; i < 64; ++i) acc[i] = 0.f;
+      convert(x, 0, ha, la);
+      load_chunk(1, x);
 #pragma unroll 1
-    for (int kc = 0; kc < nchunks; kc += 2) {
-      const uint32_t s0 = mma_chunk(ha, la, kc);
-      convert(x, kc + 1, hb, lb);
-      if (kc + 2 < nchunks) load_chunk(kc + 2, x);
-      else if (live(next_tile)) { open_tile(next_tile); load_chunk(0, x); }
-      wg_wait0();
-      fence_acc(acc);
-      w_release(s0);
-      const uint32_t s1 = mma_chunk(hb, lb, kc + 1);
-      if (kc + 2 < nchunks) { convert(x, kc + 2, ha, la); load_chunk(kc + 3, x); }
-      wg_wait0();
-      fence_acc(acc);
-      w_release(s1);
-    }
-    if (do_scores) {
-      unsigned long long best[CT];
-#pragma unroll
-      for (int k = 0; k < CT; ++k) best[k] = 0ull;
-#pragma unroll
-      for (int i = 0; i < 2; ++i) {
-        const uint32_t n = t_row + 8 * i;
+      for (int kc = 0; kc < nchunks; kc += 2) {
+        const uint32_t s0 = mma_chunk(ha, la, kc);
+        convert(x, kc + 1, hb, lb);
+        if (kc + 2 < nchunks) load_chunk(kc + 2, x);
+        else if (ATTEND ? next_tile >= 0 : live(next_tile)) { open_tile(next_tile); load_chunk(0, x); }
+        wg_wait0();
+        fence_acc(acc);
+        w_release(s0);
+        const uint32_t s1 = mma_chunk(hb, lb, kc + 1);
+        if (kc + 2 < nchunks) { convert(x, kc + 2, ha, la); load_chunk(kc + 3, x); }
+        wg_wait0();
+        fence_acc(acc);
+        w_release(s1);
+      }
+      if (do_scores) {
+        unsigned long long best[CT];
+#pragma unroll
+        for (int k = 0; k < CT; ++k) best[k] = 0ull;
+#pragma unroll
+        for (int i = 0; i < 2; ++i) {
+          const uint32_t n = t_row + 8 * i;
+#pragma unroll
+          for (int k = 0; k < CT; ++k) {
+            float v = sc[i][k];
+            v += __shfl_xor_sync(0xffffffffu, v, 2);
+            v += __shfl_xor_sync(0xffffffffu, v, 1);
+            if (q == 0 && k < C && n < t_N) {
+              v += a.bi[k];
+              a.classes[(t_rowoff + n) * C + k] = v;
+              const unsigned long long key = pack_key(v, n);
+              best[k] = key > best[k] ? key : best[k];
+            }
+          }
+        }
 #pragma unroll
         for (int k = 0; k < CT; ++k) {
-          float v = sc[i][k];
-          v += __shfl_xor_sync(0xffffffffu, v, 2);
-          v += __shfl_xor_sync(0xffffffffu, v, 1);
-          if (q == 0 && k < C && n < t_N) {
-            v += a.bi[k];
-            a.classes[(t_rowoff + n) * C + k] = v;
-            const unsigned long long key = pack_key(v, n);
-            best[k] = key > best[k] ? key : best[k];
+          const unsigned long long b = warp_max_u64(best[k]);
+          if (lane == 0 && k < C && b) atomicMax(a.keys + static_cast<size_t>(my_bag) * kMaxC + k, b);
+        }
+      }
+      uint32_t h2[32], l2[32];
+#pragma unroll
+      for (int j = 0; j < 16; ++j) {
+        const float2 bb = *reinterpret_cast<const float2*>(&s_b1[8 * j + 2 * q]);
+#pragma unroll
+        for (int i = 0; i < 2; ++i) {
+          const float h0 = fmaxf(acc[4 * j + 2 * i] + bb.x, 0.f), h1 = fmaxf(acc[4 * j + 2 * i + 1] + bb.y, 0.f);
+          if (a.H1 != nullptr && t_row + 8 * i < t_N)
+            *reinterpret_cast<float2*>(a.H1 + (t_rowoff + t_row + 8 * i) * kQ + 8 * j + 2 * q) = make_float2(h0, h1);
+          const __nv_bfloat162 hh = __floats2bfloat162_rn(h0, h1);
+          const uint32_t hu = *reinterpret_cast<const uint32_t*>(&hh);
+          const __nv_bfloat162 ll = __floats2bfloat162_rn(h0 - __uint_as_float(hu << 16), h1 - __uint_as_float(hu & 0xffff0000u));
+          h2[4 * (j >> 1) + 2 * (j & 1) + i] = hu;
+          l2[4 * (j >> 1) + 2 * (j & 1) + i] = *reinterpret_cast<const uint32_t*>(&ll);
+        }
+      }
+      float qa[64];
+#pragma unroll
+      for (int i = 0; i < 64; ++i) qa[i] = 0.f;
+      const uint32_t w0 = w_next(), w1 = w_next();
+      {
+        const uint64_t b0 = smem_desc(wring + w0 * kChunkBytes), b1 = smem_desc(wring + w1 * kChunkBytes);
+        wg_fence();
+#pragma unroll
+        for (int s = 0; s < 8; ++s) {
+          const uint64_t bh = (s < 4 ? b0 : b1) + 2 * (s & 3), bl = bh + (kTileBytes >> 4);
+          mma_rs(qa, h2[4 * s], h2[4 * s + 1], h2[4 * s + 2], h2[4 * s + 3], bh, s > 0);
+          mma_rs(qa, l2[4 * s], l2[4 * s + 1], l2[4 * s + 2], l2[4 * s + 3], bh, 1);
+          mma_rs(qa, h2[4 * s], h2[4 * s + 1], h2[4 * s + 2], h2[4 * s + 3], bl, 1);
+        }
+        wg_commit();
+        wg_wait0();
+        fence_acc(qa);
+        w_release(w0);
+        w_release(w1);
+      }
+#pragma unroll
+      for (int j = 0; j < 16; ++j) {
+        const int c = 8 * j + 2 * q;
+        const float2 bb = *reinterpret_cast<const float2*>(&s_b2[c]);
+#pragma unroll
+        for (int i = 0; i < 2; ++i) {
+          const float z0 = qa[4 * j + 2 * i] + bb.x, z1 = qa[4 * j + 2 * i + 1] + bb.y;
+          if (a.q_blocked) {
+            float* dst = a.Q + static_cast<size_t>(tile) * (kTileM * kQ) + static_cast<size_t>(c) * kTileM + rloc + 8 * i;
+            dst[0] = z0;
+            dst[kTileM] = z1;
+          } else if (t_row + 8 * i < t_N) {
+            *reinterpret_cast<float2*>(a.Q + (t_rowoff + t_row + 8 * i) * kQ + c) = make_float2(tanh_ex2(z0), tanh_ex2(z1));
           }
         }
       }
-#pragma unroll
-      for (int k = 0; k < CT; ++k) {
-        const unsigned long long b = warp_max_u64(best[k]);
-        if (lane == 0 && k < C && b) atomicMax(a.keys + static_cast<size_t>(my_bag) * kMaxC + k, b);
-      }
-    }
-    uint32_t h2[32], l2[32];
-#pragma unroll
-    for (int j = 0; j < 16; ++j) {
-      const float2 bb = *reinterpret_cast<const float2*>(&s_b1[8 * j + 2 * q]);
-#pragma unroll
-      for (int i = 0; i < 2; ++i) {
-        const float h0 = fmaxf(acc[4 * j + 2 * i] + bb.x, 0.f), h1 = fmaxf(acc[4 * j + 2 * i + 1] + bb.y, 0.f);
-        if (a.H1 != nullptr && t_row + 8 * i < t_N)
-          *reinterpret_cast<float2*>(a.H1 + (t_rowoff + t_row + 8 * i) * kQ + 8 * j + 2 * q) = make_float2(h0, h1);
-        const __nv_bfloat162 hh = __floats2bfloat162_rn(h0, h1);
-        const uint32_t hu = *reinterpret_cast<const uint32_t*>(&hh);
-        const __nv_bfloat162 ll = __floats2bfloat162_rn(h0 - __uint_as_float(hu << 16), h1 - __uint_as_float(hu & 0xffff0000u));
-        h2[4 * (j >> 1) + 2 * (j & 1) + i] = hu;
-        l2[4 * (j >> 1) + 2 * (j & 1) + i] = *reinterpret_cast<const uint32_t*>(&ll);
-      }
-    }
-    float qa[64];
-#pragma unroll
-    for (int i = 0; i < 64; ++i) qa[i] = 0.f;
-    const uint32_t w0 = w_next(), w1 = w_next();
-    {
-      const uint64_t b0 = smem_desc(wring + w0 * kChunkBytes), b1 = smem_desc(wring + w1 * kChunkBytes);
-      wg_fence();
-#pragma unroll
-      for (int s = 0; s < 8; ++s) {
-        const uint64_t bh = (s < 4 ? b0 : b1) + 2 * (s & 3), bl = bh + (kTileBytes >> 4);
-        mma_rs(qa, h2[4 * s], h2[4 * s + 1], h2[4 * s + 2], h2[4 * s + 3], bh, s > 0);
-        mma_rs(qa, l2[4 * s], l2[4 * s + 1], l2[4 * s + 2], l2[4 * s + 3], bh, 1);
-        mma_rs(qa, h2[4 * s], h2[4 * s + 1], h2[4 * s + 2], h2[4 * s + 3], bl, 1);
-      }
-      wg_commit();
-      wg_wait0();
-      fence_acc(qa);
-      w_release(w0);
-      w_release(w1);
-    }
-#pragma unroll
-    for (int j = 0; j < 16; ++j) {
-      const int c = 8 * j + 2 * q;
-      const float2 bb = *reinterpret_cast<const float2*>(&s_b2[c]);
-#pragma unroll
-      for (int i = 0; i < 2; ++i) {
-        const float z0 = qa[4 * j + 2 * i] + bb.x, z1 = qa[4 * j + 2 * i + 1] + bb.y;
-        if (a.q_blocked) {
-          float* dst = a.Q + static_cast<size_t>(tile) * (kTileM * kQ) + static_cast<size_t>(c) * kTileM + rloc + 8 * i;
-          dst[0] = z0;
-          dst[kTileM] = z1;
-        } else if (t_row + 8 * i < t_N) {
-          *reinterpret_cast<float2*>(a.Q + (t_rowoff + t_row + 8 * i) * kQ + c) = make_float2(tanh_ex2(z0), tanh_ex2(z1));
-        }
-      }
-    }
-    tile = next_tile;
+      if constexpr (ATTEND) {
+        __threadfence();
+        ConsumerSync::sync();
+        if (tid == 0) atomicAdd(att.done + my_bag, 1u);
+      }
+      tile = next_tile;
+    }
+    if constexpr (ATTEND) {
+      if (rpos >= 0) {
+        constexpr int NJ = DT == 512 ? 1 : (CT == 4 ? 2 : 4);
+        const int bag = uc.seg - 1;
+        const BagDev bg = tbl[bag];
+        if (tid == 0) wait_count(att.done + bag, static_cast<unsigned int>(uc.tiles(bag)));
+        ConsumerSync::sync();
+        const AttendArgs aa{a.bags, a.nb, D, C, a.Q, true, a.keys, att.A, att.recs, nullptr, nullptr};
+        float* s_att = sWi + CT * D;
+        constexpr bool PRE = CT == 1 || (DT == 512 && CT <= 2);
+        attend_record<CT, NJ, ConsumerSync, true, PRE>(
+            aa, bag, bg, bg.rec_off + rpos, s_att + CT * (kQ + 2 * kAttRows + 8), reinterpret_cast<float(*)[kQ]>(s_att),
+            reinterpret_cast<float(*)[CT]>(s_att + CT * kQ), reinterpret_cast<float(*)[CT]>(s_att + CT * (kQ + kAttRows)),
+            reinterpret_cast<float(*)[CT]>(s_att + CT * (kQ + 2 * kAttRows)));
+      }
+      unit += gridDim.x;
+    }
   }
 }
 
@@ -457,7 +787,7 @@
   auto go = [&](auto kern) -> int {
     DSMIL_CUDA_OK(cudaFuncSetAttribute(kern, cudaFuncAttributeMaxDynamicSharedMemorySize, static_cast<int>(smem)));
     prof_begin(PROF_FUSED, st);
-    kern<<<grid, kThreads, smem, st>>>(a);
+    kern<<<grid, kThreads, smem, st>>>(a, AttendOut{});
     prof_end(PROF_FUSED, st);
     DSMIL_LAUNCH_OK("k_qmlp_sm90");
     return 0;
```

Result: no change. 381.7 million, median of 6 (-1.2%).
